# OpenGVLab/MM-Interleaved

Hardware: NVIDIA H100
Metric: interleaved_steps_per_sec (higher is better)
Workload: dtype bf16

## Files before the change

include/mmfs_b200.h:

```cpp
#ifndef MMFS_B200_H_
#define MMFS_B200_H_

#include <stdint.h>

#ifdef __cplusplus
extern "C" {
#endif

#define MMFS_B200_ABI_VERSION 3

#define MMFS_OK            0
#define MMFS_EINVAL       (-1)
#define MMFS_EUNSUPPORTED (-2)
#define MMFS_ECUDA        (-3)

#define MMFS_F32  0
#define MMFS_F16  1
#define MMFS_BF16 2
#define MMFS_F64  3

#define MMFS_MSDA_STRICT 1u

#define MMFS_SAMPLER_EXACT_WEIGHTS 4u
#define MMFS_SAMPLER_GENERIC       8u

int mmfs_abi_version(void);
const char *mmfs_last_error(void);

int mmfs_msda_forward(const void *value, const int64_t *spatial_shapes, const int64_t *level_start,
                      const void *sampling_loc, const void *attn_weight, void *out,
                      int N, int S, int M, int D, int L, int Lq, int P,
                      int dtype, unsigned flags, void *stream);

int mmfs_msda_backward(const void *value, const int64_t *spatial_shapes, const int64_t *level_start,
                       const void *sampling_loc, const void *attn_weight, const void *grad_out,
                       float *grad_value, float *grad_loc, float *grad_attn,
                       int N, int S, int M, int D, int L, int Lq, int P, int dtype, void *stream);

int mmfs_msda_backward_deterministic(const void *value, const int64_t *spatial_shapes, const int64_t *level_start,
                                     const void *sampling_loc, const void *attn_weight, const void *grad_out,
                                     long long *grad_value_fixed, float *grad_value, float *grad_loc, float *grad_attn,
                                     float *scratch2, int N, int S, int M, int D, int L, int Lq, int P, int dtype, void *stream);

int mmfs_msda_index_stream(const int64_t *spatial_shapes, const int64_t *level_start,
                           const void *sampling_loc, int32_t *idx,
                           int N, int M, int D, int L, int Lq, int P,
                           int dtype, void *stream);

int mmfs_msda_forward_host(const void *value, const int64_t *spatial_shapes, const int64_t *level_start,
                           const void *sampling_loc, const void *attn_weight, void *out,
                           int N, int S, int M, int D, int L, int Lq, int P,
                           int dtype, unsigned flags, void *stream);
void mmfs_release_scratch(void);

int mmfs_sampler_forward(const void *value, const int64_t *shapes, const int64_t *starts,
                         const void *qproj, const void *rtable, const uint8_t *relpos,
                         const float *refpts, const float *scale_ratios, void *out, float *null_mass,
                         int N, int S, int M, int D, int n_img, int n_lvl, int Lq, int P,
                         int Lq_r, int Nr, int Lr, int R, int dtype, unsigned flags, void *stream);

int mmfs_sampler_locw(const int64_t *shapes, const int64_t *starts, const void *qproj, const void *rtable,
                      const uint8_t *relpos, const float *refpts, const float *scale_ratios,
                      void *loc_out, void *attn_out, float *null_mass,
                      int N, int M, int n_img, int n_lvl, int Lq, int P,
                      int Lq_r, int Nr, int Lr, int R, int dtype, void *stream);

int mmfs_rmsnorm(const void *x, const void *weight, void *y, long rows, int cols, float eps, int dtype, void *stream);
int mmfs_layernorm(const void *x, const void *weight, const void *bias, void *y, long rows, int cols, float eps,
                   int dtype, void *stream);
int mmfs_rope_qk(void *q, void *k, const float *cos_table, const float *sin_table, const int64_t *position_ids,
                 long n_tokens, int T_len, int H, int hd, int q_stride, int k_stride, int pos_per_batch,
                 int dtype, void *stream);
int mmfs_rope_qk_append(void *q, const void *k, const void *v, const float *cos_table, const float *sin_table,
                        const int64_t *position_ids, void *k_cache, void *v_cache, const int64_t *slot_dev, long slot_host,
                        long n_tokens, int T_len, int H, int hd, int q_stride, int k_stride, int v_stride, long cache_bs,
                        long cache_ts, int pos_per_batch, int dtype, void *stream);
int mmfs_swiglu(const void *gate_up, void *out, long rows, int inter, int dtype, void *stream);
int mmfs_geglu(const void *value_gate, void *out, long rows, int inter, int dtype, void *stream);

int mmfs_attn_generic(const void *q, const void *k, const void *v, void *out, const uint8_t *key_mask,
                      int B, int H, int Tq, int Tkv, int hd,
                      long q_bs, long q_ts, long k_bs, long k_ts, long v_bs, long v_ts, long o_bs, long o_ts,
                      float scale, int causal, int past, int dtype, void *stream);
long mmfs_attn_decode_scratch_floats(int B, int H, int Tkv, int hd);
int mmfs_attn_decode(const void *q, const void *k, const void *v, void *out, const uint8_t *key_mask, float *scratch,
                     int B, int H, int Tkv, int hd, long q_bs, long k_bs, long k_ts, long v_bs, long v_ts, long o_bs,
                     float scale, int causal, int past, int dtype, void *stream);

int mmfs_attn_forward(const void *q, const void *k, const void *v, void *out, const uint8_t *key_mask,
                      int B, int H, int Tq, int Tkv, int hd,
                      long q_bs, long q_ts, long k_bs, long k_ts, long v_bs, long v_ts, long o_bs, long o_ts,
                      float scale, int causal, int past, int dtype, unsigned *work_counter, void *stream);

int mmfs_attn_forward_lse(const void *q, const void *k, const void *v, void *out, float *lse, const uint8_t *key_mask,
                          int B, int H, int Tq, int Tkv, int hd,
                          long q_bs, long q_ts, long k_bs, long k_ts, long v_bs, long v_ts, long o_bs, long o_ts,
                          float scale, int causal, int past, int dtype, unsigned *work_counter, void *stream);

int mmfs_attn_backward(const void *q, const void *k, const void *v, const void *out, const void *d_out, const float *lse,
                       void *dq, void *dk, void *dv, float *delta, const uint8_t *key_mask, int B, int H, int T, int hd,
                       long q_bs, long q_ts, long k_bs, long k_ts, long v_bs, long v_ts, long o_bs, long o_ts,
                       long do_bs, long do_ts, long dq_bs, long dq_ts, long dk_bs, long dk_ts, long dv_bs, long dv_ts,
                       float scale, int dtype, void *stream);

#define MMFS_RMSNORM_BWD_PARTS 256
int mmfs_rmsnorm_backward(const void *x, const void *weight, const void *dy, void *dx, void *dweight, float *partials,
                          long rows, int cols, float eps, int dtype, void *stream);

int mmfs_swiglu_backward(const void *gate_up, const void *d_out, void *d_gate_up, long rows, int inter, int dtype,
                         void *stream);

int mmfs_conv2d_nhwc(const void *x, const void *w, const void *bias, const void *add_bc, const void *residual, void *out,
                     int B, int H, int W, int Cin, int Cout, int KH, int KW, int stride, int pad, int dtype, void *stream);

int mmfs_conv2d_up2x_nhwc(const void *x, const void *w_phases, const void *bias, void *out, int B, int H, int W, int Cin,
                          int Cout, int dtype, void *stream);

int mmfs_conv2d_down2x_nhwc(const void *x, const void *w, const void *bias, void *out, int B, int H, int W, int Cin,
                            int Cout, int dtype, void *stream);

int mmfs_groupnorm_nhwc(const void *x, const void *gamma, const void *beta, void *y, float *stats, int B, int HW, int C,
                        int G, float eps, int silu, int dtype, void *stream);

#define MMFS_SELECT_GREEDY 0
#define MMFS_SELECT_SAMPLE 1

int mmfs_decode_select(const float *logits, long ld, int64_t *out_ids, const int64_t *step, uint8_t *finished,
                       int64_t *next_ids, const int64_t *eos_ids, int n_eos, long pad_id, int min_length,
                       const float *params, const int64_t *seed, const float *uniforms, int B, int V, int max_new,
                       int mode, void *stream);

int mmfs_beam_select(const float *logits, long ld, const int64_t *step, const double *params, float *beam_scores,
                     int64_t *history, int64_t *next_ids, int64_t *parent, uint8_t *done, double *hyp_scores,
                     int64_t *hyp_ids, int64_t *hyp_meta, const int64_t *eos_ids, int n_eos, long pad_id, int min_length,
                     uint64_t *scratch, int B, int num_beams, int V, int max_new, void *stream);

int mmfs_beam_sample(const float *logits, long ld, const int64_t *step, const double *params, const int64_t *seed,
                     const float *uniforms, float *beam_scores, int64_t *history, int64_t *next_ids, int64_t *parent,
                     uint8_t *done, double *hyp_scores, int64_t *hyp_ids, int64_t *hyp_meta, int32_t *error,
                     const int64_t *eos_ids, int n_eos, long pad_id, int min_length, int top_k, uint64_t *scratch, int B,
                     int num_beams, int V, int max_new, void *stream);

int mmfs_kv_beam_reorder(void *cache, int n_caches, long cache_stride, int rows, long row_stride, long pos_stride,
                         long row_bytes, int num_beams, const int64_t *parent, const int64_t *cur, const int64_t *step,
                         const uint8_t *done, int max_positions, void *stream);

#ifdef __cplusplus
}
#endif
#endif
```

mm-interleaved_b200/_lib.py:

```python
from __future__ import annotations

import ctypes
import os

_HERE = os.path.dirname(os.path.abspath(__file__))
LIB_PATH = os.environ.get("MMFS_B200_LIB", os.path.join(_HERE, "libmmfs_b200.so"))

OK, EINVAL, EUNSUPPORTED, ECUDA = 0, -1, -2, -3
F32, F16, BF16, F64 = 0, 1, 2, 3
MSDA_STRICT = 1
SAMPLER_EXACT_WEIGHTS = 4
SAMPLER_GENERIC = 8
SELECT_GREEDY, SELECT_SAMPLE = 0, 1

_lib = None

_I, _U, _P = ctypes.c_int, ctypes.c_uint, ctypes.c_void_p
_L, _F = ctypes.c_long, ctypes.c_float

SIGNATURES = {
    "mmfs_abi_version": (_I, []),
    "mmfs_last_error": (ctypes.c_char_p, []),
    "mmfs_msda_forward": (_I, [_P, _P, _P, _P, _P, _P, _I, _I, _I, _I, _I, _I, _I, _I, _U, _P]),
    "mmfs_msda_backward": (_I, [_P] * 9 + [_I] * 8 + [_P]),
    "mmfs_msda_backward_deterministic": (_I, [_P] * 11 + [_I] * 8 + [_P]),
    "mmfs_msda_index_stream": (_I, [_P, _P, _P, _P, _I, _I, _I, _I, _I, _I, _I, _P]),
    "mmfs_msda_forward_host": (_I, [_P, _P, _P, _P, _P, _P, _I, _I, _I, _I, _I, _I, _I, _I, _U, _P]),
    "mmfs_release_scratch": (None, []),
    "mmfs_sampler_forward": (_I, [_P] * 10 + [_I] * 13 + [_U, _P]),
    "mmfs_sampler_locw": (_I, [_P] * 10 + [_I] * 11 + [_P]),
    "mmfs_rmsnorm": (_I, [_P, _P, _P, _L, _I, _F, _I, _P]),
    "mmfs_layernorm": (_I, [_P, _P, _P, _P, _L, _I, _F, _I, _P]),
    "mmfs_rope_qk": (_I, [_P, _P, _P, _P, _P, _L, _I, _I, _I, _I, _I, _I, _I, _P]),
    "mmfs_rope_qk_append": (_I, [_P] * 9 + [_L, _L] + [_I] * 6 + [_L, _L, _I, _I, _P]),
    "mmfs_swiglu": (_I, [_P, _P, _L, _I, _I, _P]),
    "mmfs_geglu": (_I, [_P, _P, _L, _I, _I, _P]),
    "mmfs_attn_generic": (_I, [_P] * 5 + [_I] * 5 + [_L] * 8 + [_F, _I, _I, _I, _P]),
    "mmfs_groupnorm_nhwc": (_I, [_P] * 5 + [_I] * 4 + [_F, _I, _I, _P]),
    "mmfs_conv2d_nhwc": (_I, [_P] * 6 + [_I] * 10 + [_P]),
    "mmfs_conv2d_up2x_nhwc": (_I, [_P] * 4 + [_I] * 6 + [_P]),
    "mmfs_conv2d_down2x_nhwc": (_I, [_P] * 4 + [_I] * 6 + [_P]),
    "mmfs_attn_decode_scratch_floats": (_L, [_I] * 4),
    "mmfs_attn_decode": (_I, [_P] * 6 + [_I] * 4 + [_L] * 6 + [_F, _I, _I, _I, _P]),
    "mmfs_attn_forward": (_I, [_P] * 5 + [_I] * 5 + [_L] * 8 + [_F, _I, _I, _I, _P, _P]),
    "mmfs_attn_forward_lse": (_I, [_P] * 6 + [_I] * 5 + [_L] * 8 + [_F, _I, _I, _I, _P, _P]),
    "mmfs_attn_backward": (_I, [_P] * 11 + [_I] * 4 + [_L] * 16 + [_F, _I, _P]),
    "mmfs_rmsnorm_backward": (_I, [_P] * 6 + [_L, _I, _F, _I, _P]),
    "mmfs_swiglu_backward": (_I, [_P] * 3 + [_L, _I, _I, _P]),
    "mmfs_decode_select": (_I, [_P, _L] + [_P] * 5 + [_I, _L, _I] + [_P] * 3 + [_I] * 4 + [_P]),
    "mmfs_beam_select": (_I, [_P, _L] + [_P] * 11 + [_I, _L, _I, _P] + [_I] * 4 + [_P]),
    "mmfs_beam_sample": (_I, [_P, _L] + [_P] * 14 + [_I, _L, _I, _I, _P] + [_I] * 4 + [_P]),
    "mmfs_kv_beam_reorder": (_I, [_P, _I, _L, _I, _L, _L, _L, _I] + [_P] * 4 + [_I, _P]),
}
BEAM_MAX_BEAMS, BEAM_MAX_EOS = 8, 4
RMSNORM_BWD_PARTS = 256


def lib() -> ctypes.CDLL:
    global _lib
    if _lib is None:
        if not os.path.exists(LIB_PATH):
            raise RuntimeError(
                f"libmmfs_b200.so not found at {LIB_PATH}: build it with "
                "`python mm-interleaved_b200/build.py` (there is no CPU / PyTorch fallback)")
        handle = ctypes.CDLL(LIB_PATH)
        for name, (res, args) in SIGNATURES.items():
            fn = getattr(handle, name)
            fn.restype = res
            fn.argtypes = args
        if handle.mmfs_abi_version() != 3:
            raise RuntimeError(f"libmmfs_b200.so ABI {handle.mmfs_abi_version()} != 3")
        _lib = handle
    return _lib


def check(rc: int, what: str) -> None:
    if rc != OK:
        msg = lib().mmfs_last_error().decode("utf-8", "replace")
        kind = {EINVAL: "invalid argument", EUNSUPPORTED: "unsupported", ECUDA: "CUDA error"}.get(rc, "error")
        raise RuntimeError(f"{what}: {kind} ({rc}): {msg}")
```

mm-interleaved_b200/csrc/conv_igemm_sm100.cu:

```cuda
#include "tc_common.cuh"

namespace mmfs {

constexpr int kConvStages = 4;
constexpr int kConvThreads = 288;
constexpr int kConvConsumers = 256;

struct ConvParams {
    void *out;
    const void *bias, *add_bc, *residual;
    int B, Ho, Wo, Cin, Cout, KH, KW, stride, pad;
    int TW, TH, TB;
    int tiles_w, tiles_h;
};

template <typename T> __device__ __forceinline__ uint32_t cpack2(float a, float b);
template <> __device__ __forceinline__ uint32_t cpack2<__nv_bfloat16>(float a, float b) {
    __nv_bfloat162 t = __floats2bfloat162_rn(a, b);
    return *reinterpret_cast<uint32_t *>(&t);
}
template <> __device__ __forceinline__ uint32_t cpack2<__half>(float a, float b) {
    __half2 t = __floats2half2_rn(a, b);
    return *reinterpret_cast<uint32_t *>(&t);
}
template <typename T> __device__ __forceinline__ float2 cunpack2(const T *p);
template <> __device__ __forceinline__ float2 cunpack2<__nv_bfloat16>(const __nv_bfloat16 *p) {
    return __bfloat1622float2(*reinterpret_cast<const __nv_bfloat162 *>(p));
}
template <> __device__ __forceinline__ float2 cunpack2<__half>(const __half *p) {
    return __half22float2(*reinterpret_cast<const __half2 *>(p));
}

template <typename T, int BN, bool UP>
__global__ void __launch_bounds__(kConvThreads, 1)
conv_igemm_kernel(const __grid_constant__ CUtensorMap map_x, const __grid_constant__ CUtensorMap map_w, const ConvParams p) {
    static_assert(BN == 160 || BN == 128, "Cout tile");
    constexpr uint32_t A_BYTES = 128 * 128, B_BYTES = BN * 128, STAGE_BYTES = A_BYTES + B_BYTES;
    extern __shared__ __align__(1024) uint8_t smem_raw[];
    if ((s_addr(smem_raw) & 1023u) != 0u) { asm volatile("trap;"); }
    uint64_t *bars = reinterpret_cast<uint64_t *>(smem_raw + kConvStages * STAGE_BYTES);
    uint64_t *full = bars, *empty = bars + kConvStages;

    const int warp = threadIdx.x >> 5, lane = threadIdx.x & 31;
    int t = blockIdx.x;
    const int wt = t % p.tiles_w; t /= p.tiles_w;
    const int ht = t % p.tiles_h; t /= p.tiles_h;
    const int b0 = t * p.TB, h0 = ht * p.TH, w0 = wt * p.TW;
    const int n0 = blockIdx.y * BN;
    const int kc = p.Cin / 64;
    const int n_k = p.KH * p.KW * kc;

    if (threadIdx.x == 0) {
        for (int i = 0; i < kConvStages; ++i) { bar_init(full + i, 1); bar_init(empty + i, kConvConsumers); }
        asm volatile("fence.mbarrier_init.release.cluster;" ::: "memory");
    }
    __syncthreads();

    if (warp == 8) {
        if (lane == 0) {
            for (int it = 0; it < n_k; ++it) {
                const int s = it % kConvStages;
                const uint32_t ph = (it / kConvStages) & 1;
                bar_wait(empty + s, ph ^ 1);
                const int tap = it / kc, cb = it - tap * kc;
                const int kh = tap / p.KW, kw = tap - kh * p.KW;
                uint8_t *sa = smem_raw + s * STAGE_BYTES;
                bar_expect_tx(full + s, STAGE_BYTES);
                if constexpr (UP) {
                    const int phase = blockIdx.z;
                    tma_load_4d(sa, &map_x, full + s, cb * 64, w0 + kw - 1 + (phase & 1), h0 + kh - 1 + (phase >> 1), b0);
                    tma_load_2d(sa + A_BYTES, &map_w, full + s, tap * p.Cin + cb * 64, phase * p.Cout + n0);
                } else {
                    tma_load_4d(sa, &map_x, full + s, cb * 64, w0 * p.stride + kw - p.pad, h0 * p.stride + kh - p.pad, b0);
                    tma_load_2d(sa + A_BYTES, &map_w, full + s, tap * p.Cin + cb * 64, n0);
                }
            }
        }
        return;
    }

    const int wg = warp >> 2;
    float acc[BN / 2];
#pragma unroll
    for (int i = 0; i < BN / 2; ++i) acc[i] = 0.f;
    for (int it = 0; it < n_k; ++it) {
        const int s = it % kConvStages;
        bar_wait(full + s, (it / kConvStages) & 1);
        const uint32_t sa = s_addr(smem_raw) + s * STAGE_BYTES;
        reg_fence(acc);
        wgmma_fence();
#pragma unroll
        for (int kk = 0; kk < 4; ++kk) {
            const uint64_t da = smem_desc(sa + wg * 64 * 128 + kk * 32, 16, 1024), db = smem_desc(sa + A_BYTES + kk * 32, 16, 1024);
            if constexpr (BN == 160) Wgmma<T>::ss_n160(acc, da, db, 1);
            else Wgmma<T>::ss_n128(acc, da, db, 1);
        }
        wgmma_commit();
        wgmma_wait<1>();
        reg_fence(acc);
        if (it > 0) bar_arrive(empty + (it - 1) % kConvStages);
    }
    wgmma_wait<0>();
    reg_fence(acc);

    const int tq = lane & 3;
    const T *bp = p.bias ? static_cast<const T *>(p.bias) + n0 + 2 * tq : nullptr;
#pragma unroll
    for (int i = 0; i < 2; ++i) {
        const int row = wg * 64 + (warp & 3) * 16 + (lane >> 2) + 8 * i;
        const int pw = row % p.TW, phh = (row / p.TW) % p.TH, pb = row / (p.TW * p.TH);
        const int b = b0 + pb, ho = h0 + phh, wo = w0 + pw;
        if (b >= p.B || ho >= p.Ho || wo >= p.Wo) continue;
        size_t pix;
        if constexpr (UP) pix = ((size_t)b * 2 * p.Ho + 2 * ho + (blockIdx.z >> 1)) * 2 * p.Wo + 2 * wo + (blockIdx.z & 1);
        else pix = ((size_t)b * p.Ho + ho) * p.Wo + wo;
        T *op = static_cast<T *>(p.out) + pix * p.Cout + n0 + 2 * tq;
        const T *rp = p.residual ? static_cast<const T *>(p.residual) + pix * p.Cout + n0 + 2 * tq : nullptr;
        const T *ap = p.add_bc ? static_cast<const T *>(p.add_bc) + (size_t)b * p.Cout + n0 + 2 * tq : nullptr;
#pragma unroll
        for (int j = 0; j < BN / 8; ++j) {
            float e0 = acc[j * 4 + 2 * i], e1 = acc[j * 4 + 2 * i + 1];
            if (bp) { const float2 f = cunpack2<T>(bp + j * 8); e0 += f.x; e1 += f.y; }
            if (ap) { const float2 f = cunpack2<T>(ap + j * 8); e0 += f.x; e1 += f.y; }
            if (rp) { const float2 f = cunpack2<T>(rp + j * 8); e0 += f.x; e1 += f.y; }
            *reinterpret_cast<uint32_t *>(op + j * 8) = cpack2<T>(e0, e1);
        }
    }
}

}

using namespace mmfs;

namespace {

int conv_bn(int Cout) { return Cout % 160 == 0 ? 160 : Cout % 128 == 0 ? 128 : 0; }

template <auto kern>
int launch(dim3 grid, size_t smem, cudaStream_t st, const CUtensorMap &mx, const CUtensorMap &mw, const ConvParams &p) {
    const int rc = ensure_dynamic_smem<kern>(smem);
    if (rc != MMFS_OK) return rc;
    kern<<<grid, kConvThreads, smem, st>>>(mx, mw, p);
    MMFS_CUDA(cudaGetLastError());
    return MMFS_OK;
}

template <bool UP>
int launch_conv(const char *what, const void *x, const void *w, const void *bias, const void *add_bc, const void *residual,
                void *out, int B, int H, int W, int Ho, int Wo, int Cin, int Cout, int KH, int KW, int stride, int pad,
                int dtype, void *stream) {
    int TW, TH, TB;
    if (Wo % 16 == 0 && Ho % 8 == 0) { TW = 16; TH = 8; TB = 1; }
    else if (Wo == 8 && Ho == 8 && B % 2 == 0) { TW = 8; TH = 8; TB = 2; }
    else { set_error("%s: output %dx%d (B=%d) is not tileable by the 128-pixel patches", what, Ho, Wo, B); return MMFS_EUNSUPPORTED; }
    const int BN = conv_bn(Cout);
    if (!(dtype == MMFS_BF16 || dtype == MMFS_F16) || Cin % 64 != 0 || BN == 0 || stride > 2 ||
        ((uintptr_t)x | (uintptr_t)w | (uintptr_t)out | (uintptr_t)bias | (uintptr_t)add_bc | (uintptr_t)residual) % 16 != 0) {
        set_error("%s: needs bf16/f16, Cin %% 64 == 0, Cout %% 160 == 0 or Cout %% 128 == 0, stride <= 2, 16-byte aligned "
                  "pointers (Cin=%d Cout=%d)", what, Cin, Cout);
        return MMFS_EUNSUPPORTED;
    }
    EncodeTiledFn enc = tensor_map_encoder();
    if (!enc) { set_error("%s: cuTensorMapEncodeTiled unavailable", what); return MMFS_ECUDA; }
    const CUtensorMapDataType dt = dtype == MMFS_BF16 ? CU_TENSOR_MAP_DATA_TYPE_BFLOAT16 : CU_TENSOR_MAP_DATA_TYPE_FLOAT16;
    const int phases = UP ? 4 : 1;
    CUtensorMap mx, mw;
    {
        const cuuint64_t dims[4] = {(cuuint64_t)Cin, (cuuint64_t)W, (cuuint64_t)H, (cuuint64_t)B};
        const cuuint64_t strides[3] = {(cuuint64_t)Cin * 2, (cuuint64_t)W * Cin * 2, (cuuint64_t)H * W * Cin * 2};
        const cuuint32_t box[4] = {64, (cuuint32_t)(TW * stride), (cuuint32_t)(TH * stride), (cuuint32_t)TB};
        const cuuint32_t estr[4] = {1, (cuuint32_t)stride, (cuuint32_t)stride, 1};
        CUresult r = enc(&mx, dt, 4, const_cast<void *>(x), dims, strides, box, estr, CU_TENSOR_MAP_INTERLEAVE_NONE,
                         CU_TENSOR_MAP_SWIZZLE_128B, CU_TENSOR_MAP_L2_PROMOTION_L2_128B, CU_TENSOR_MAP_FLOAT_OOB_FILL_NONE);
        if (r != CUDA_SUCCESS) { set_error("%s: tensor map (input) failed (%d)", what, (int)r); return MMFS_ECUDA; }
    }
    {
        const cuuint64_t K = (cuuint64_t)KH * KW * Cin;
        const cuuint64_t dims[2] = {K, (cuuint64_t)Cout * phases};
        const cuuint64_t strides[1] = {K * 2};
        const cuuint32_t box[2] = {64, (cuuint32_t)BN};
        const cuuint32_t estr[2] = {1, 1};
        CUresult r = enc(&mw, dt, 2, const_cast<void *>(w), dims, strides, box, estr, CU_TENSOR_MAP_INTERLEAVE_NONE,
                         CU_TENSOR_MAP_SWIZZLE_128B, CU_TENSOR_MAP_L2_PROMOTION_L2_256B, CU_TENSOR_MAP_FLOAT_OOB_FILL_NONE);
        if (r != CUDA_SUCCESS) { set_error("%s: tensor map (weights) failed (%d)", what, (int)r); return MMFS_ECUDA; }
    }
    ConvParams p;
    p.out = out; p.bias = bias; p.add_bc = add_bc; p.residual = residual;
    p.B = B; p.Ho = Ho; p.Wo = Wo; p.Cin = Cin; p.Cout = Cout; p.KH = KH; p.KW = KW; p.stride = stride; p.pad = pad;
    p.TW = TW; p.TH = TH; p.TB = TB; p.tiles_w = Wo / TW; p.tiles_h = Ho / TH;
    const size_t smem = (size_t)kConvStages * (128 * 128 + BN * 128) + 2 * kConvStages * 8;
    dim3 grid((unsigned)(p.tiles_w * p.tiles_h * (B / TB)), (unsigned)(Cout / BN), (unsigned)phases);
    cudaStream_t st = (cudaStream_t)stream;
    return dispatch_dtype<kF16Types>(dtype, what, [&](auto tag) {
        using T = typename decltype(tag)::type;
        return BN == 160 ? launch<conv_igemm_kernel<T, 160, UP>>(grid, smem, st, mx, mw, p)
                         : launch<conv_igemm_kernel<T, 128, UP>>(grid, smem, st, mx, mw, p);
    });
}

}

extern "C" int mmfs_conv2d_nhwc(const void *x, const void *w, const void *bias, const void *add_bc, const void *residual, void *out,
                                int B, int H, int W, int Cin, int Cout, int KH, int KW, int stride, int pad,
                                int dtype, void *stream) {
    MMFS_CHECK_ARG(B > 0 && H > 0 && W > 0 && Cin > 0 && Cout > 0 && KH > 0 && KW > 0 && stride > 0 && pad >= 0, "conv2d_nhwc: bad dimension");
    MMFS_CHECK_ARG(x && w && out, "conv2d_nhwc: null pointer argument");
    const int Ho = (H + 2 * pad - KH) / stride + 1, Wo = (W + 2 * pad - KW) / stride + 1;
    return launch_conv<false>("conv2d_nhwc", x, w, bias, add_bc, residual, out, B, H, W, Ho, Wo, Cin, Cout, KH, KW, stride,
                              pad, dtype, stream);
}

extern "C" int mmfs_conv2d_up2x_nhwc(const void *x, const void *w_phases, const void *bias, void *out, int B, int H, int W, int Cin,
                                     int Cout, int dtype, void *stream) {
    MMFS_CHECK_ARG(B > 0 && H > 0 && W > 0 && Cin > 0 && Cout > 0, "conv2d_up2x_nhwc: bad dimension");
    MMFS_CHECK_ARG(x && w_phases && out, "conv2d_up2x_nhwc: null pointer argument");
    return launch_conv<true>("conv2d_up2x_nhwc", x, w_phases, bias, nullptr, nullptr, out, B, H, W, H, W, Cin, Cout, 2, 2, 1, 0,
                             dtype, stream);
}

extern "C" int mmfs_conv2d_down2x_nhwc(const void *x, const void *w, const void *bias, void *out, int B, int H, int W, int Cin,
                                       int Cout, int dtype, void *stream) {
    MMFS_CHECK_ARG(B > 0 && H > 0 && W > 0 && Cin > 0 && Cout > 0, "conv2d_down2x_nhwc: bad dimension");
    MMFS_CHECK_ARG(x && w && out, "conv2d_down2x_nhwc: null pointer argument");
    MMFS_CHECK_ARG(H % 2 == 0 && W % 2 == 0, "conv2d_down2x_nhwc: odd H or W");
    return launch_conv<false>("conv2d_down2x_nhwc", x, w, bias, nullptr, nullptr, out, B, H, W, H / 2, W / 2, Cin, Cout, 3, 3,
                              2, 0, dtype, stream);
}
```

mm-interleaved_b200/csrc/llama_ops_sm100.cu:

```cuda
#include "common.cuh"

namespace mmfs {

template <typename T> __device__ __forceinline__ float rnd(float x) { return to_op(from_op<T>(x)); }
template <> __device__ __forceinline__ float rnd<float>(float x) { return x; }

__device__ __forceinline__ float block_sum(float v, float *s_red) {
#pragma unroll
    for (int o = 16; o > 0; o >>= 1) v += __shfl_xor_sync(0xffffffffu, v, o);
    const int lane = threadIdx.x & 31, warp = threadIdx.x >> 5, nw = (blockDim.x + 31) >> 5;
    if (lane == 0) s_red[warp] = v;
    __syncthreads();
    float t = (lane < nw) ? s_red[lane] : 0.f;
#pragma unroll
    for (int o = 16; o > 0; o >>= 1) t += __shfl_xor_sync(0xffffffffu, t, o);
    __syncthreads();
    return t;
}

template <typename T>
__global__ void __launch_bounds__(256) rmsnorm_kernel(const T *__restrict__ x, const T *__restrict__ w,
                                                       T *__restrict__ y, int cols, float eps) {
    constexpr int VEC = 16 / (int)sizeof(T);
    __shared__ float s_red[32];
    const size_t row = blockIdx.x;
    const T *xr = x + row * cols;
    T *yr = y + row * cols;
    const int nvec = cols / VEC;
    float ss = 0.f;
    for (int i = threadIdx.x; i < nvec; i += blockDim.x) {
        float f[VEC];
        Vec16<T>::unpack(*reinterpret_cast<const uint4 *>(xr + i * VEC), f);
#pragma unroll
        for (int k = 0; k < VEC; ++k) ss += f[k] * f[k];
    }
    for (int i = nvec * VEC + threadIdx.x; i < cols; i += blockDim.x) { const float v = to_op(xr[i]); ss += v * v; }
    const float var = block_sum(ss, s_red) / (float)cols;
    const float r = rsqrtf(var + eps);
    for (int i = threadIdx.x; i < nvec; i += blockDim.x) {
        float f[VEC], g[VEC], o[VEC];
        Vec16<T>::unpack(*reinterpret_cast<const uint4 *>(xr + i * VEC), f);
        Vec16<T>::unpack(*reinterpret_cast<const uint4 *>(w + i * VEC), g);
#pragma unroll
        for (int k = 0; k < VEC; ++k) o[k] = g[k] * rnd<T>(f[k] * r);
        *reinterpret_cast<uint4 *>(yr + i * VEC) = Vec16<T>::pack(o);
    }
    for (int i = nvec * VEC + threadIdx.x; i < cols; i += blockDim.x)
        yr[i] = from_op<T>(to_op(w[i]) * rnd<T>(to_op(xr[i]) * r));
}

constexpr int kRmsChunks = 8;
constexpr int kRmsThreads = 128;

template <typename T>
__global__ void __launch_bounds__(kRmsThreads) rmsnorm_reg_kernel(const T *__restrict__ x, const T *__restrict__ w,
                                                                  T *__restrict__ y, int cols, float eps) {
    constexpr int VEC = 16 / (int)sizeof(T);
    __shared__ float s_red[kRmsThreads / 32];
    const size_t row = blockIdx.x;
    const T *xr = x + row * cols;
    T *yr = y + row * cols;
    const int nvec = cols / VEC;
    uint4 v[kRmsChunks], wv[kRmsChunks];
#pragma unroll
    for (int c = 0; c < kRmsChunks; ++c) {
        const int i = threadIdx.x + c * kRmsThreads;
        if (i < nvec) {
            v[c] = ldg_nc_v4(xr + i * VEC);
            wv[c] = ldg_nc_v4(w + i * VEC);
        }
    }
    float ss = 0.f;
#pragma unroll
    for (int c = 0; c < kRmsChunks; ++c)
        if (threadIdx.x + c * kRmsThreads < nvec) {
            float f[VEC];
            Vec16<T>::unpack(v[c], f);
#pragma unroll
            for (int k = 0; k < VEC; ++k) ss = fmaf(f[k], f[k], ss);
        }
#pragma unroll
    for (int o = 16; o > 0; o >>= 1) ss += __shfl_xor_sync(0xffffffffu, ss, o);
    if ((threadIdx.x & 31) == 0) s_red[threadIdx.x >> 5] = ss;
    __syncthreads();
    float tot = 0.f;
#pragma unroll
    for (int i = 0; i < kRmsThreads / 32; ++i) tot += s_red[i];
    const float r = rsqrtf(tot / (float)cols + eps);
#pragma unroll
    for (int c = 0; c < kRmsChunks; ++c) {
        const int i = threadIdx.x + c * kRmsThreads;
        if (i < nvec) {
            float f[VEC], g[VEC], o[VEC];
            Vec16<T>::unpack(v[c], f);
            Vec16<T>::unpack(wv[c], g);
#pragma unroll
            for (int k = 0; k < VEC; ++k) o[k] = g[k] * rnd<T>(f[k] * r);
            stg_v4(yr + i * VEC, Vec16<T>::pack(o));
        }
    }
}

constexpr int kLnChunks = 8;

template <typename T, int CH>
__global__ void __launch_bounds__(256, CH == 8 ? 2 : 4) layernorm_warp_kernel(const T *__restrict__ x, const T *__restrict__ w,
                                                              const T *__restrict__ b, T *__restrict__ y, long rows, int cols, float eps) {
    constexpr int VEC = 16 / (int)sizeof(T);
    const int lane = threadIdx.x & 31;
    const long row = (long)blockIdx.x * (blockDim.x >> 5) + (threadIdx.x >> 5);
    if (row >= rows) return;
    const T *xr = x + row * cols;
    T *yr = y + row * cols;
    const int nvec = cols / VEC;
    uint4 v[CH];
#pragma unroll
    for (int c = 0; c < CH; ++c) {
        const int i = lane + 32 * c;
        v[c] = (i < nvec) ? ldg_nc_v4(xr + i * VEC) : make_uint4(0u, 0u, 0u, 0u);
    }
    float s = 0.f;
#pragma unroll
    for (int c = 0; c < CH; ++c) {
        float f[VEC];
        Vec16<T>::unpack(v[c], f);
#pragma unroll
        for (int k = 0; k < VEC; ++k) s += f[k];
    }
#pragma unroll
    for (int o = 16; o > 0; o >>= 1) s += __shfl_xor_sync(0xffffffffu, s, o);
    const float mean = s / (float)cols;
    float ss = 0.f;
#pragma unroll
    for (int c = 0; c < CH; ++c)
        if (lane + 32 * c < nvec) {
            float f[VEC];
            Vec16<T>::unpack(v[c], f);
#pragma unroll
            for (int k = 0; k < VEC; ++k) { const float d = f[k] - mean; ss = fmaf(d, d, ss); }
        }
#pragma unroll
    for (int o = 16; o > 0; o >>= 1) ss += __shfl_xor_sync(0xffffffffu, ss, o);
    const float r = rsqrtf(ss / (float)cols + eps);
#pragma unroll
    for (int c = 0; c < CH; ++c) {
        const int i = lane + 32 * c;
        if (i < nvec) {
            float f[VEC], g[VEC], bb[VEC], o[VEC];
            Vec16<T>::unpack(v[c], f);
            if (w) Vec16<T>::unpack(*reinterpret_cast<const uint4 *>(w + i * VEC), g);
            if (b) Vec16<T>::unpack(*reinterpret_cast<const uint4 *>(b + i * VEC), bb);
#pragma unroll
            for (int k = 0; k < VEC; ++k) o[k] = (f[k] - mean) * r * (w ? g[k] : 1.f) + (b ? bb[k] : 0.f);
            stg_v4(yr + i * VEC, Vec16<T>::pack(o));
        }
    }
}

template <typename T>
__global__ void __launch_bounds__(256) layernorm_kernel(const T *__restrict__ x, const T *__restrict__ w,
                                                         const T *__restrict__ b, T *__restrict__ y, int cols, float eps) {
    __shared__ float s_red[32];
    const size_t row = blockIdx.x;
    const T *xr = x + row * cols;
    T *yr = y + row * cols;
    float s = 0.f;
    for (int i = threadIdx.x; i < cols; i += blockDim.x) s += to_op(xr[i]);
    const float mean = block_sum(s, s_red) / (float)cols;
    float ss = 0.f;
    for (int i = threadIdx.x; i < cols; i += blockDim.x) { const float d = to_op(xr[i]) - mean; ss += d * d; }
    const float r = rsqrtf(block_sum(ss, s_red) / (float)cols + eps);
    for (int i = threadIdx.x; i < cols; i += blockDim.x) {
        const float n = (to_op(xr[i]) - mean) * r;
        yr[i] = from_op<T>(n * (w ? to_op(w[i]) : 1.f) + (b ? to_op(b[i]) : 0.f));
    }
}

template <typename T>
__global__ void __launch_bounds__(256) rope_qk_kernel(T *__restrict__ q, T *__restrict__ k, const float *__restrict__ cos_t,
                                                       const float *__restrict__ sin_t, const int64_t *__restrict__ pos,
                                                       long n_tok, int H, int hd, int q_stride, int k_stride, int pos_per_batch,
                                                       int T_len) {
    constexpr int VEC = 16 / (int)sizeof(T);
    const int half = hd >> 1;
    const int chunks = half / VEC;
    const int per_tok = 2 * H * chunks;
    const bool hoist = (blockDim.x % chunks) == 0;
    for (long tok = blockIdx.x; tok < n_tok; tok += gridDim.x) {
        const long p = pos[pos_per_batch ? tok : (tok % T_len)];
        const float *cp = cos_t + p * hd, *sp = sin_t + p * hd;
        T *qt = q + tok * q_stride, *kt = k + tok * k_stride;
        float cs[VEC], sn[VEC];
        auto load_table = [&](int c) {
#pragma unroll
            for (int i = 0; i < VEC; i += 4) {
                const float4 a = *reinterpret_cast<const float4 *>(cp + c * VEC + i);
                const float4 b = *reinterpret_cast<const float4 *>(sp + c * VEC + i);
                cs[i] = rnd<T>(a.x); cs[i + 1] = rnd<T>(a.y); cs[i + 2] = rnd<T>(a.z); cs[i + 3] = rnd<T>(a.w);
                sn[i] = rnd<T>(b.x); sn[i + 1] = rnd<T>(b.y); sn[i + 2] = rnd<T>(b.z); sn[i + 3] = rnd<T>(b.w);
            }
        };
        if (hoist) load_table(threadIdx.x % chunks);
        for (int it = threadIdx.x; it < per_tok; it += blockDim.x) {
            const int c = it % chunks;
            const int hh = it / chunks;
            T *x = (hh >= H ? kt + (size_t)(hh - H) * hd : qt + (size_t)hh * hd) + c * VEC;
            float x1[VEC], x2[VEC], o1[VEC], o2[VEC];
            const uint4 v1 = *reinterpret_cast<const uint4 *>(x), v2 = *reinterpret_cast<const uint4 *>(x + half);
            if (!hoist) load_table(c);
            Vec16<T>::unpack(v1, x1);
            Vec16<T>::unpack(v2, x2);
#pragma unroll
            for (int i = 0; i < VEC; ++i) {
                o1[i] = rnd<T>(x1[i] * cs[i]) + rnd<T>(-x2[i] * sn[i]);
                o2[i] = rnd<T>(x2[i] * cs[i]) + rnd<T>(x1[i] * sn[i]);
            }
            *reinterpret_cast<uint4 *>(x) = Vec16<T>::pack(o1);
            *reinterpret_cast<uint4 *>(x + half) = Vec16<T>::pack(o2);
        }
    }
}

template <typename T>
__global__ void __launch_bounds__(256) rope_append_kernel(T *__restrict__ q, const T *__restrict__ k, const T *__restrict__ v,
                                                           const float *__restrict__ cos_t, const float *__restrict__ sin_t,
                                                           const int64_t *__restrict__ pos, T *__restrict__ k_cache,
                                                           T *__restrict__ v_cache, const int64_t *__restrict__ slot_dev,
                                                           long slot_host, long n_tok, int H, int hd, int q_stride, int k_stride,
                                                           int v_stride, long cache_bs, long cache_ts, int pos_per_batch, int T_len) {
    constexpr int VEC = 16 / (int)sizeof(T);
    const int half = hd >> 1;
    const int chunks = half / VEC;
    const int n_rot = 2 * H * chunks;
    const int n_copy = H * hd / VEC;
    const long slot = slot_dev != nullptr ? (long)*slot_dev : slot_host;
    for (long tok = blockIdx.x; tok < n_tok; tok += gridDim.x) {
        const long p = pos[pos_per_batch ? tok : (tok % T_len)];
        const float *cp = cos_t + p * hd, *sp = sin_t + p * hd;
        const long b = tok / T_len, tt = tok - b * T_len;
        T *qt = q + tok * q_stride;
        const T *kt = k + tok * k_stride, *vt = v + tok * v_stride;
        T *kc = k_cache + b * cache_bs + (slot + tt) * cache_ts, *vc = v_cache + b * cache_bs + (slot + tt) * cache_ts;
        for (int it = threadIdx.x; it < n_rot + n_copy; it += blockDim.x) {
            if (it >= n_rot) {
                const int i = (it - n_rot) * VEC;
                *reinterpret_cast<uint4 *>(vc + i) = *reinterpret_cast<const uint4 *>(vt + i);
                continue;
            }
            const int c = it % chunks, hh = it / chunks;
            const bool is_k = hh >= H;
            const T *src = (is_k ? kt + (size_t)(hh - H) * hd : qt + (size_t)hh * hd) + c * VEC;
            T *dst = (is_k ? kc + (size_t)(hh - H) * hd : qt + (size_t)hh * hd) + c * VEC;
            float cs[VEC], sn[VEC], x1[VEC], x2[VEC], o1[VEC], o2[VEC];
#pragma unroll
            for (int i = 0; i < VEC; i += 4) {
                const float4 a = *reinterpret_cast<const float4 *>(cp + c * VEC + i);
                const float4 bb = *reinterpret_cast<const float4 *>(sp + c * VEC + i);
                cs[i] = rnd<T>(a.x); cs[i + 1] = rnd<T>(a.y); cs[i + 2] = rnd<T>(a.z); cs[i + 3] = rnd<T>(a.w);
                sn[i] = rnd<T>(bb.x); sn[i + 1] = rnd<T>(bb.y); sn[i + 2] = rnd<T>(bb.z); sn[i + 3] = rnd<T>(bb.w);
            }
            Vec16<T>::unpack(*reinterpret_cast<const uint4 *>(src), x1);
            Vec16<T>::unpack(*reinterpret_cast<const uint4 *>(src + half), x2);
#pragma unroll
            for (int i = 0; i < VEC; ++i) {
                o1[i] = rnd<T>(x1[i] * cs[i]) + rnd<T>(-x2[i] * sn[i]);
                o2[i] = rnd<T>(x2[i] * cs[i]) + rnd<T>(x1[i] * sn[i]);
            }
            *reinterpret_cast<uint4 *>(dst) = Vec16<T>::pack(o1);
            *reinterpret_cast<uint4 *>(dst + half) = Vec16<T>::pack(o2);
        }
    }
}

template <typename T> __device__ __forceinline__ float silu_op(float g) { return __fdividef(g, 1.f + __expf(-g)); }
template <> __device__ __forceinline__ float silu_op<float>(float g) { return g / (1.f + expf(-g)); }

template <typename T, int ACT> __device__ __forceinline__ float glu_act(float g) {
    if (ACT == 0) return silu_op<T>(g);
    return 0.5f * g * (1.f + erff(g * 0.70710678118654752f));
}

template <typename T, int ACT = 0, bool GATE_SECOND = false>
__global__ void __launch_bounds__(256) swiglu_kernel(const T *__restrict__ gu, T *__restrict__ out, long rows, int I) {
    constexpr int VEC = 16 / (int)sizeof(T);
    const int per = (I / VEC + gridDim.y - 1) / gridDim.y;
    const int v0 = blockIdx.y * per, nvec = min(I / VEC, v0 + per);
    for (long r = blockIdx.x; r < rows; r += gridDim.x) {
        const T *g_row = gu + r * 2 * I + (GATE_SECOND ? I : 0), *u_row = gu + r * 2 * I + (GATE_SECOND ? 0 : I);
        T *o_row = out + r * I;
        int i = v0 + threadIdx.x;
        for (; i + (int)blockDim.x < nvec; i += 2 * blockDim.x) {
            const int j = i + blockDim.x;
            const uint4 g0 = ldg_nc_v4(g_row + i * VEC), u0 = ldg_nc_v4(u_row + i * VEC);
            const uint4 g1 = ldg_nc_v4(g_row + j * VEC), u1 = ldg_nc_v4(u_row + j * VEC);
            float g[VEC], u[VEC], o[VEC];
            Vec16<T>::unpack(g0, g); Vec16<T>::unpack(u0, u);
#pragma unroll
            for (int k = 0; k < VEC; ++k) o[k] = rnd<T>(glu_act<T, ACT>(g[k])) * u[k];
            stg_v4(o_row + i * VEC, Vec16<T>::pack(o));
            Vec16<T>::unpack(g1, g); Vec16<T>::unpack(u1, u);
#pragma unroll
            for (int k = 0; k < VEC; ++k) o[k] = rnd<T>(glu_act<T, ACT>(g[k])) * u[k];
            stg_v4(o_row + j * VEC, Vec16<T>::pack(o));
        }
        if (i < nvec) {
            float g[VEC], u[VEC], o[VEC];
            Vec16<T>::unpack(ldg_nc_v4(g_row + i * VEC), g); Vec16<T>::unpack(ldg_nc_v4(u_row + i * VEC), u);
#pragma unroll
            for (int k = 0; k < VEC; ++k) o[k] = rnd<T>(glu_act<T, ACT>(g[k])) * u[k];
            stg_v4(o_row + i * VEC, Vec16<T>::pack(o));
        }
    }
}

template <typename T>
static int launch_rmsnorm(const void *x, const void *w, void *y, long rows, int cols, float eps, cudaStream_t st) {
    if (cols % (16 / (int)sizeof(T)) == 0 && cols / (16 / (int)sizeof(T)) <= kRmsThreads * kRmsChunks)
        rmsnorm_reg_kernel<T><<<(unsigned)rows, kRmsThreads, 0, st>>>((const T *)x, (const T *)w, (T *)y, cols, eps);
    else
        rmsnorm_kernel<T><<<(unsigned)rows, 256, 0, st>>>((const T *)x, (const T *)w, (T *)y, cols, eps);
    MMFS_CUDA(cudaGetLastError());
    return MMFS_OK;
}

template <typename T>
static int launch_layernorm(const void *x, const void *w, const void *b, void *y, long rows, int cols, float eps, cudaStream_t st) {
    constexpr int VEC = 16 / (int)sizeof(T);
    const bool vec_ok = (cols % VEC == 0) && (cols / VEC <= 32 * kLnChunks) &&
                        (((uintptr_t)x | (uintptr_t)y | (uintptr_t)w | (uintptr_t)b) % 16 == 0);
    if (vec_ok) {
        const int nvec = cols / VEC;
        const unsigned grid = (unsigned)((rows + 7) / 8);
#define MMFS_LN(CH) layernorm_warp_kernel<T, CH><<<grid, 256, 0, st>>>((const T *)x, (const T *)w, (const T *)b, (T *)y, rows, cols, eps)
        if (nvec <= 32) MMFS_LN(1); else if (nvec <= 64) MMFS_LN(2); else if (nvec <= 128) MMFS_LN(4); else MMFS_LN(8);
#undef MMFS_LN
    } else
        layernorm_kernel<T><<<(unsigned)rows, 256, 0, st>>>((const T *)x, (const T *)w, (const T *)b, (T *)y, cols, eps);
    MMFS_CUDA(cudaGetLastError());
    return MMFS_OK;
}

template <typename T>
static int launch_rope(void *q, void *k, const float *cos_t, const float *sin_t, const int64_t *pos, long n_tok, int T_len,
                       int H, int hd, int qs, int ks, int ppb, cudaStream_t st) {
    const int per_tok = H * 2 * ((hd / 2) / (16 / (int)sizeof(T)));
    const int threads = per_tok >= 256 ? 256 : ((per_tok + 31) / 32) * 32;
    rope_qk_kernel<T><<<capped_grid(n_tok, 32), threads, 0, st>>>((T *)q, (T *)k, cos_t, sin_t, pos, n_tok, H, hd, qs, ks, ppb,
                                                                  T_len);
    MMFS_CUDA(cudaGetLastError());
    return MMFS_OK;
}

template <typename T>
static int launch_glu(const void *in, void *out, long rows, int inter, bool geglu, cudaStream_t st) {
    const int nvec = inter / (16 / (int)sizeof(T));
    const int threads = nvec >= 512 ? 256 : (nvec >= 64 ? 64 : 32);
    const int gx = capped_grid(rows, 64);
    int gy = 1;
    if (gx < num_sms()) { gy = (nvec + 2 * threads - 1) / (2 * threads); if (gy > 64) gy = 64; if (gy < 1) gy = 1; }
    const dim3 grid(gx, gy);
    if (geglu)
        swiglu_kernel<T, 1, true><<<grid, threads, 0, st>>>((const T *)in, (T *)out, rows, inter);
    else
        swiglu_kernel<T, 0, false><<<grid, threads, 0, st>>>((const T *)in, (T *)out, rows, inter);
    MMFS_CUDA(cudaGetLastError());
    return MMFS_OK;
}

template <typename T>
static int launch_rope_append(void *q, const void *k, const void *v, const float *cos_t, const float *sin_t, const int64_t *pos,
                              void *kc, void *vc, const int64_t *slot_dev, long slot_host, long n_tok, int T_len, int H, int hd,
                              int qs, int ks, int vs, long cbs, long cts, int ppb, cudaStream_t st) {
    const int items = H * ((hd / 2) / (16 / (int)sizeof(T))) * 2 + H * hd / (16 / (int)sizeof(T));
    const int threads = items >= 256 ? 256 : ((items + 31) / 32) * 32;
    rope_append_kernel<T><<<capped_grid(n_tok, 32), threads, 0, st>>>((T *)q, (const T *)k, (const T *)v, cos_t, sin_t, pos, (T *)kc,
                                                                      (T *)vc, slot_dev, slot_host, n_tok, H, hd, qs, ks, vs, cbs,
                                                                      cts, ppb, T_len);
    MMFS_CUDA(cudaGetLastError());
    return MMFS_OK;
}


constexpr int kRmsBwdParts = MMFS_RMSNORM_BWD_PARTS;
constexpr int kRmsBwdMaxCols = 8192;

template <typename T>
__global__ void __launch_bounds__(256) rmsnorm_bwd_kernel(const T *__restrict__ x, const T *__restrict__ w,
                                                          const T *__restrict__ dy, T *__restrict__ dx,
                                                          float *__restrict__ partials, long rows, int cols, float eps) {
    constexpr int VEC = 16 / (int)sizeof(T);
    extern __shared__ float s_dw[];
    __shared__ float s_red[32];
    const int nvec = cols / VEC;
    if (partials)
        for (int i = threadIdx.x; i < nvec; i += blockDim.x)
#pragma unroll
            for (int k = 0; k < VEC; ++k) s_dw[i * VEC + k] = 0.f;
    for (long row = blockIdx.x; row < rows; row += gridDim.x) {
        const T *xr = x + row * cols, *dyr = dy + row * cols;
        float ss = 0.f, sg = 0.f;
        for (int i = threadIdx.x; i < nvec; i += blockDim.x) {
            float f[VEC], g[VEC], d[VEC];
            Vec16<T>::unpack(ldg_nc_v4(xr + i * VEC), f);
            Vec16<T>::unpack(ldg_nc_v4(w + i * VEC), g);
            Vec16<T>::unpack(ldg_nc_v4(dyr + i * VEC), d);
#pragma unroll
            for (int k = 0; k < VEC; ++k) { ss = fmaf(f[k], f[k], ss); sg = fmaf(d[k] * g[k], f[k], sg); }
        }
        ss = block_sum(ss, s_red);
        sg = block_sum(sg, s_red);
        const float r = rsqrtf(ss / (float)cols + eps);
        const float coef = r * r * r * sg / (float)cols;
        for (int i = threadIdx.x; i < nvec; i += blockDim.x) {
            float f[VEC], g[VEC], d[VEC], o[VEC];
            Vec16<T>::unpack(ldg_nc_v4(xr + i * VEC), f);
            Vec16<T>::unpack(ldg_nc_v4(w + i * VEC), g);
            Vec16<T>::unpack(ldg_nc_v4(dyr + i * VEC), d);
#pragma unroll
            for (int k = 0; k < VEC; ++k) o[k] = fmaf(r * d[k], g[k], -f[k] * coef);
            stg_v4(dx + row * cols + i * VEC, Vec16<T>::pack(o));
            if (partials)
#pragma unroll
                for (int k = 0; k < VEC; ++k) s_dw[i * VEC + k] = fmaf(d[k], rnd<T>(f[k] * r), s_dw[i * VEC + k]);
        }
    }
    if (partials)
        for (int i = threadIdx.x; i < nvec; i += blockDim.x)
#pragma unroll
            for (int k = 0; k < VEC; ++k) partials[(long)blockIdx.x * cols + i * VEC + k] = s_dw[i * VEC + k];
}

template <typename T>
__global__ void __launch_bounds__(256) rmsnorm_dw_reduce_kernel(const float *__restrict__ partials, T *__restrict__ dw,
                                                                int parts, int cols) {
    const int c = blockIdx.x * blockDim.x + threadIdx.x;
    if (c >= cols) return;
    float s = 0.f;
    for (int p = 0; p < parts; ++p) s += partials[(long)p * cols + c];
    dw[c] = from_op<T>(s);
}

template <typename T>
__global__ void __launch_bounds__(256) swiglu_bwd_kernel(const T *__restrict__ gu, const T *__restrict__ d_out,
                                                         T *__restrict__ d_gu, long rows, int I) {
    constexpr int VEC = 16 / (int)sizeof(T);
    const int nvec = I / VEC;
    for (long r = blockIdx.x; r < rows; r += gridDim.x)
        for (int i = threadIdx.x; i < nvec; i += blockDim.x) {
            float g[VEC], u[VEC], d[VEC], dg[VEC], du[VEC];
            Vec16<T>::unpack(ldg_nc_v4(gu + r * 2 * I + i * VEC), g);
            Vec16<T>::unpack(ldg_nc_v4(gu + r * 2 * I + I + i * VEC), u);
            Vec16<T>::unpack(ldg_nc_v4(d_out + r * I + i * VEC), d);
#pragma unroll
            for (int k = 0; k < VEC; ++k) {
                const float s = 1.f / (1.f + expf(-g[k]));
                dg[k] = d[k] * u[k] * s * fmaf(g[k], 1.f - s, 1.f);
                du[k] = d[k] * g[k] * s;
            }
            stg_v4(d_gu + r * 2 * I + i * VEC, Vec16<T>::pack(dg));
            stg_v4(d_gu + r * 2 * I + I + i * VEC, Vec16<T>::pack(du));
        }
}

template <typename T>
static int launch_rmsnorm_bwd(const void *x, const void *w, const void *dy, void *dx, void *dw, float *partials, long rows,
                              int cols, float eps, cudaStream_t st) {
    const int parts = (int)(rows < kRmsBwdParts ? rows : kRmsBwdParts);
    rmsnorm_bwd_kernel<T><<<parts, 256, dw ? cols * sizeof(float) : 0, st>>>(
        (const T *)x, (const T *)w, (const T *)dy, (T *)dx, dw ? partials : nullptr, rows, cols, eps);
    MMFS_CUDA(cudaGetLastError());
    if (dw) {
        rmsnorm_dw_reduce_kernel<T><<<(cols + 255) / 256, 256, 0, st>>>(partials, (T *)dw, parts, cols);
        MMFS_CUDA(cudaGetLastError());
    }
    return MMFS_OK;
}

template <typename T>
static int launch_swiglu_bwd(const void *gu, const void *d_out, void *d_gu, long rows, int inter, cudaStream_t st) {
    swiglu_bwd_kernel<T><<<capped_grid(rows, 8), 256, 0, st>>>((const T *)gu, (const T *)d_out, (T *)d_gu, rows, inter);
    MMFS_CUDA(cudaGetLastError());
    return MMFS_OK;
}

}

using namespace mmfs;

extern "C" int mmfs_rmsnorm(const void *x, const void *weight, void *y, long rows, int cols, float eps, int dtype, void *stream) {
    MMFS_CHECK_ARG(rows >= 0 && cols > 0, "rmsnorm: bad shape");
    if (rows == 0) return MMFS_OK;
    MMFS_CHECK_ARG(x && weight && y, "rmsnorm: null pointer argument");
    MMFS_CHECK_ARG(((uintptr_t)x | (uintptr_t)weight | (uintptr_t)y) % 16 == 0 && (cols * dtype_size(dtype)) % 16 == 0,
                   "rmsnorm: rows must be 16-byte aligned");
    return dispatch_dtype<kF32Types>(dtype, "rmsnorm", [&](auto tag) {
        return launch_rmsnorm<typename decltype(tag)::type>(x, weight, y, rows, cols, eps, (cudaStream_t)stream);
    });
}

extern "C" int mmfs_layernorm(const void *x, const void *weight, const void *bias, void *y, long rows, int cols, float eps,
                              int dtype, void *stream) {
    MMFS_CHECK_ARG(rows >= 0 && cols > 0, "layernorm: bad shape");
    if (rows == 0) return MMFS_OK;
    MMFS_CHECK_ARG(x && y, "layernorm: null pointer argument");
    return dispatch_dtype<kF32Types>(dtype, "layernorm", [&](auto tag) {
        return launch_layernorm<typename decltype(tag)::type>(x, weight, bias, y, rows, cols, eps, (cudaStream_t)stream);
    });
}

extern "C" int mmfs_rope_qk(void *q, void *k, const float *cos_table, const float *sin_table, const int64_t *position_ids,
                            long n_tokens, int T_len, int H, int hd, int q_stride, int k_stride, int pos_per_batch,
                            int dtype, void *stream) {
    MMFS_CHECK_ARG(n_tokens >= 0 && H > 0 && hd > 0 && hd % 2 == 0 && T_len > 0, "rope_qk: bad shape");
    if (n_tokens == 0) return MMFS_OK;
    MMFS_CHECK_ARG(q && k && cos_table && sin_table && position_ids, "rope_qk: null pointer argument");
    MMFS_CHECK_ARG((hd / 2) % (16 / (int)dtype_size(dtype)) == 0 && ((uintptr_t)q | (uintptr_t)k) % 16 == 0 &&
                   (q_stride * dtype_size(dtype)) % 16 == 0 && (k_stride * dtype_size(dtype)) % 16 == 0,
                   "rope_qk: head_dim/2 must be a multiple of the 16-byte vector and rows 16-byte aligned");
    return dispatch_dtype<kF32Types>(dtype, "rope_qk", [&](auto tag) {
        return launch_rope<typename decltype(tag)::type>(q, k, cos_table, sin_table, position_ids, n_tokens, T_len, H, hd, q_stride,
                                                         k_stride, pos_per_batch, (cudaStream_t)stream);
    });
}

extern "C" int mmfs_rope_qk_append(void *q, const void *k, const void *v, const float *cos_table, const float *sin_table,
                                   const int64_t *position_ids, void *k_cache, void *v_cache, const int64_t *slot_dev,
                                   long slot_host, long n_tokens, int T_len, int H, int hd, int q_stride, int k_stride,
                                   int v_stride, long cache_bs, long cache_ts, int pos_per_batch, int dtype, void *stream) {
    MMFS_CHECK_ARG(n_tokens >= 0 && H > 0 && hd > 0 && hd % 2 == 0 && T_len > 0 && slot_host >= 0, "rope_qk_append: bad shape");
    if (n_tokens == 0) return MMFS_OK;
    MMFS_CHECK_ARG(q && k && v && cos_table && sin_table && position_ids && k_cache && v_cache, "rope_qk_append: null pointer argument");
    const size_t es = dtype_size(dtype);
    MMFS_CHECK_ARG(es == 2 || es == 4, "rope_qk_append: f32 / f16 / bf16");
    MMFS_CHECK_ARG((hd / 2) % (16 / (int)es) == 0 &&
                       ((uintptr_t)q | (uintptr_t)k | (uintptr_t)v | (uintptr_t)k_cache | (uintptr_t)v_cache) % 16 == 0 &&
                       (q_stride * es) % 16 == 0 && (k_stride * es) % 16 == 0 && (v_stride * es) % 16 == 0 &&
                       (cache_bs * es) % 16 == 0 && (cache_ts * es) % 16 == 0,
                   "rope_qk_append: head_dim/2 must be a multiple of the 16-byte vector and all rows 16-byte aligned");
    return dispatch_dtype<kF32Types>(dtype, "rope_qk_append", [&](auto tag) {
        return launch_rope_append<typename decltype(tag)::type>(q, k, v, cos_table, sin_table, position_ids, k_cache, v_cache,
                                                                slot_dev, slot_host, n_tokens, T_len, H, hd, q_stride, k_stride,
                                                                v_stride, cache_bs, cache_ts, pos_per_batch, (cudaStream_t)stream);
    });
}

extern "C" int mmfs_swiglu(const void *gate_up, void *out, long rows, int inter, int dtype, void *stream) {
    MMFS_CHECK_ARG(rows >= 0 && inter > 0, "swiglu: bad shape");
    if (rows == 0) return MMFS_OK;
    MMFS_CHECK_ARG(gate_up && out, "swiglu: null pointer argument");
    MMFS_CHECK_ARG(((uintptr_t)gate_up | (uintptr_t)out) % 16 == 0 && (inter * dtype_size(dtype)) % 16 == 0,
                   "swiglu: rows must be 16-byte aligned");
    return dispatch_dtype<kF32Types>(dtype, "swiglu", [&](auto tag) {
        return launch_glu<typename decltype(tag)::type>(gate_up, out, rows, inter, false, (cudaStream_t)stream);
    });
}

extern "C" int mmfs_geglu(const void *value_gate, void *out, long rows, int inter, int dtype, void *stream) {
    MMFS_CHECK_ARG(rows >= 0 && inter > 0, "geglu: bad shape");
    if (rows == 0) return MMFS_OK;
    MMFS_CHECK_ARG(value_gate && out, "geglu: null pointer argument");
    MMFS_CHECK_ARG(((uintptr_t)value_gate | (uintptr_t)out) % 16 == 0 && (inter * dtype_size(dtype)) % 16 == 0,
                   "geglu: rows must be 16-byte aligned");
    return dispatch_dtype<kF32Types>(dtype, "geglu", [&](auto tag) {
        return launch_glu<typename decltype(tag)::type>(value_gate, out, rows, inter, true, (cudaStream_t)stream);
    });
}

extern "C" int mmfs_rmsnorm_backward(const void *x, const void *weight, const void *dy, void *dx, void *dweight,
                                     float *partials, long rows, int cols, float eps, int dtype, void *stream) {
    MMFS_CHECK_ARG(rows >= 0 && cols > 0, "rmsnorm_backward: bad shape");
    if (rows == 0) return MMFS_OK;
    MMFS_CHECK_ARG(x && weight && dy && dx && (!dweight || partials), "rmsnorm_backward: null pointer argument");
    if (!(dtype == MMFS_BF16 || dtype == MMFS_F16) || cols % 8 != 0 || cols > kRmsBwdMaxCols ||
        ((uintptr_t)x | (uintptr_t)weight | (uintptr_t)dy | (uintptr_t)dx) % 16 != 0) {
        set_error("rmsnorm_backward: needs bf16 / f16, cols %% 8 == 0, cols <= %d, 16-byte aligned rows (got cols=%d dtype=%d)",
                  kRmsBwdMaxCols, cols, dtype);
        return MMFS_EUNSUPPORTED;
    }
    return dispatch_dtype<kF16Types, MMFS_EUNSUPPORTED>(dtype, "rmsnorm_backward", [&](auto tag) {
        return launch_rmsnorm_bwd<typename decltype(tag)::type>(x, weight, dy, dx, dweight, partials, rows, cols, eps,
                                                                (cudaStream_t)stream);
    });
}

extern "C" int mmfs_swiglu_backward(const void *gate_up, const void *d_out, void *d_gate_up, long rows, int inter, int dtype,
                                    void *stream) {
    MMFS_CHECK_ARG(rows >= 0 && inter > 0, "swiglu_backward: bad shape");
    if (rows == 0) return MMFS_OK;
    MMFS_CHECK_ARG(gate_up && d_out && d_gate_up, "swiglu_backward: null pointer argument");
    if (!(dtype == MMFS_BF16 || dtype == MMFS_F16) || inter % 8 != 0 ||
        ((uintptr_t)gate_up | (uintptr_t)d_out | (uintptr_t)d_gate_up) % 16 != 0) {
        set_error("swiglu_backward: needs bf16 / f16, inter %% 8 == 0 and 16-byte aligned rows (got inter=%d dtype=%d)", inter, dtype);
        return MMFS_EUNSUPPORTED;
    }
    return dispatch_dtype<kF16Types, MMFS_EUNSUPPORTED>(dtype, "swiglu_backward", [&](auto tag) {
        return launch_swiglu_bwd<typename decltype(tag)::type>(gate_up, d_out, d_gate_up, rows, inter, (cudaStream_t)stream);
    });
}
```

mm-interleaved_b200/csrc/tc_common.cuh:

```cuda
#pragma once
#include <cuda.h>

#include "common.cuh"

namespace mmfs {

__device__ __forceinline__ void tma_load_4d(void *dst, const CUtensorMap *map, uint64_t *bar, int c0, int c1, int c2, int c3) {
    asm volatile(
        "cp.async.bulk.tensor.4d.shared::cluster.global.mbarrier::complete_tx::bytes [%0], [%1, {%3, %4, %5, %6}], [%2];" ::
        "r"(s_addr(dst)), "l"(map), "r"(s_addr(bar)), "r"(c0), "r"(c1), "r"(c2), "r"(c3) : "memory");
}
__device__ __forceinline__ void fence_async_smem() { asm volatile("fence.proxy.async.shared::cta;" ::: "memory"); }

__device__ __forceinline__ void wgmma_fence() { asm volatile("wgmma.fence.sync.aligned;" ::: "memory"); }
__device__ __forceinline__ void wgmma_commit() { asm volatile("wgmma.commit_group.sync.aligned;" ::: "memory"); }
template <int N> __device__ __forceinline__ void wgmma_wait() { asm volatile("wgmma.wait_group.sync.aligned %0;" ::"n"(N) : "memory"); }
template <int N> __device__ __forceinline__ void reg_fence(float (&d)[N]) {
#pragma unroll
    for (int i = 0; i < N; ++i) asm volatile("" : "+f"(d[i])::"memory");
}

__device__ __forceinline__ uint64_t smem_desc(uint32_t saddr, uint32_t lbo_bytes, uint32_t sbo_bytes) {
    return (uint64_t)((saddr >> 4) & 0x3fffu) | ((uint64_t)((lbo_bytes >> 4) & 0x3fffu) << 16) |
           ((uint64_t)((sbo_bytes >> 4) & 0x3fffu) << 32) | (1ull << 62);
}

template <typename T> struct Wgmma;
#define MMFS_WGMMA_OPS(TY) \
     \
    __device__ __forceinline__ static void ss_n64(float (&d)[32], uint64_t da, uint64_t db, int acc) { \
        asm volatile( \
            "{\n\t.reg .pred p;\n\tsetp.ne.b32 p, %34, 0;\n\t" \
            "wgmma.mma_async.sync.aligned.m64n64k16.f32." TY "." TY " {%0,%1,%2,%3,%4,%5,%6,%7,%8,%9,%10,%11,%12,%13,%14,%15,%16,%17,%18,%19,%20,%21,%22,%23,%24,%25,%26,%27,%28,%29,%30,%31}, %32, %33, p, 1, 1, 0, 0;\n\t}" \
            : "+f"(d[0]), "+f"(d[1]), "+f"(d[2]), "+f"(d[3]), "+f"(d[4]), "+f"(d[5]), "+f"(d[6]), "+f"(d[7]), "+f"(d[8]), "+f"(d[9]), "+f"(d[10]), "+f"(d[11]), "+f"(d[12]), "+f"(d[13]), "+f"(d[14]), "+f"(d[15]), "+f"(d[16]), "+f"(d[17]), "+f"(d[18]), "+f"(d[19]), "+f"(d[20]), "+f"(d[21]), "+f"(d[22]), "+f"(d[23]), "+f"(d[24]), "+f"(d[25]), "+f"(d[26]), "+f"(d[27]), "+f"(d[28]), "+f"(d[29]), "+f"(d[30]), "+f"(d[31]) \
            : "l"(da), "l"(db), "r"(acc)); \
    } \
     \
    __device__ __forceinline__ static void ss_n128(float (&d)[64], uint64_t da, uint64_t db, int acc) { \
        asm volatile( \
            "{\n\t.reg .pred p;\n\tsetp.ne.b32 p, %66, 0;\n\t" \
            "wgmma.mma_async.sync.aligned.m64n128k16.f32." TY "." TY " {%0,%1,%2,%3,%4,%5,%6,%7,%8,%9,%10,%11,%12,%13,%14,%15,%16,%17,%18,%19,%20,%21,%22,%23,%24,%25,%26,%27,%28,%29,%30,%31,%32,%33,%34,%35,%36,%37,%38,%39,%40,%41,%42,%43,%44,%45,%46,%47,%48,%49,%50,%51,%52,%53,%54,%55,%56,%57,%58,%59,%60,%61,%62,%63}, %64, %65, p, 1, 1, 0, 0;\n\t}" \
            : "+f"(d[0]), "+f"(d[1]), "+f"(d[2]), "+f"(d[3]), "+f"(d[4]), "+f"(d[5]), "+f"(d[6]), "+f"(d[7]), "+f"(d[8]), "+f"(d[9]), "+f"(d[10]), "+f"(d[11]), "+f"(d[12]), "+f"(d[13]), "+f"(d[14]), "+f"(d[15]), "+f"(d[16]), "+f"(d[17]), "+f"(d[18]), "+f"(d[19]), "+f"(d[20]), "+f"(d[21]), "+f"(d[22]), "+f"(d[23]), "+f"(d[24]), "+f"(d[25]), "+f"(d[26]), "+f"(d[27]), "+f"(d[28]), "+f"(d[29]), "+f"(d[30]), "+f"(d[31]), "+f"(d[32]), "+f"(d[33]), "+f"(d[34]), "+f"(d[35]), "+f"(d[36]), "+f"(d[37]), "+f"(d[38]), "+f"(d[39]), "+f"(d[40]), "+f"(d[41]), "+f"(d[42]), "+f"(d[43]), "+f"(d[44]), "+f"(d[45]), "+f"(d[46]), "+f"(d[47]), "+f"(d[48]), "+f"(d[49]), "+f"(d[50]), "+f"(d[51]), "+f"(d[52]), "+f"(d[53]), "+f"(d[54]), "+f"(d[55]), "+f"(d[56]), "+f"(d[57]), "+f"(d[58]), "+f"(d[59]), "+f"(d[60]), "+f"(d[61]), "+f"(d[62]), "+f"(d[63]) \
            : "l"(da), "l"(db), "r"(acc)); \
    } \
     \
    __device__ __forceinline__ static void ss_n160(float (&d)[80], uint64_t da, uint64_t db, int acc) { \
        asm volatile( \
            "{\n\t.reg .pred p;\n\tsetp.ne.b32 p, %82, 0;\n\t" \
            "wgmma.mma_async.sync.aligned.m64n160k16.f32." TY "." TY " {%0,%1,%2,%3,%4,%5,%6,%7,%8,%9,%10,%11,%12,%13,%14,%15,%16,%17,%18,%19,%20,%21,%22,%23,%24,%25,%26,%27,%28,%29,%30,%31,%32,%33,%34,%35,%36,%37,%38,%39,%40,%41,%42,%43,%44,%45,%46,%47,%48,%49,%50,%51,%52,%53,%54,%55,%56,%57,%58,%59,%60,%61,%62,%63,%64,%65,%66,%67,%68,%69,%70,%71,%72,%73,%74,%75,%76,%77,%78,%79}, %80, %81, p, 1, 1, 0, 0;\n\t}" \
            : "+f"(d[0]), "+f"(d[1]), "+f"(d[2]), "+f"(d[3]), "+f"(d[4]), "+f"(d[5]), "+f"(d[6]), "+f"(d[7]), "+f"(d[8]), "+f"(d[9]), "+f"(d[10]), "+f"(d[11]), "+f"(d[12]), "+f"(d[13]), "+f"(d[14]), "+f"(d[15]), "+f"(d[16]), "+f"(d[17]), "+f"(d[18]), "+f"(d[19]), "+f"(d[20]), "+f"(d[21]), "+f"(d[22]), "+f"(d[23]), "+f"(d[24]), "+f"(d[25]), "+f"(d[26]), "+f"(d[27]), "+f"(d[28]), "+f"(d[29]), "+f"(d[30]), "+f"(d[31]), "+f"(d[32]), "+f"(d[33]), "+f"(d[34]), "+f"(d[35]), "+f"(d[36]), "+f"(d[37]), "+f"(d[38]), "+f"(d[39]), "+f"(d[40]), "+f"(d[41]), "+f"(d[42]), "+f"(d[43]), "+f"(d[44]), "+f"(d[45]), "+f"(d[46]), "+f"(d[47]), "+f"(d[48]), "+f"(d[49]), "+f"(d[50]), "+f"(d[51]), "+f"(d[52]), "+f"(d[53]), "+f"(d[54]), "+f"(d[55]), "+f"(d[56]), "+f"(d[57]), "+f"(d[58]), "+f"(d[59]), "+f"(d[60]), "+f"(d[61]), "+f"(d[62]), "+f"(d[63]), "+f"(d[64]), "+f"(d[65]), "+f"(d[66]), "+f"(d[67]), "+f"(d[68]), "+f"(d[69]), "+f"(d[70]), "+f"(d[71]), "+f"(d[72]), "+f"(d[73]), "+f"(d[74]), "+f"(d[75]), "+f"(d[76]), "+f"(d[77]), "+f"(d[78]), "+f"(d[79]) \
            : "l"(da), "l"(db), "r"(acc)); \
    } \
     \
    __device__ __forceinline__ static void rs_n64(float (&d)[32], const uint32_t (&a)[4], uint64_t db, int acc) { \
        asm volatile( \
            "{\n\t.reg .pred p;\n\tsetp.ne.b32 p, %37, 0;\n\t" \
            "wgmma.mma_async.sync.aligned.m64n64k16.f32." TY "." TY " {%0,%1,%2,%3,%4,%5,%6,%7,%8,%9,%10,%11,%12,%13,%14,%15,%16,%17,%18,%19,%20,%21,%22,%23,%24,%25,%26,%27,%28,%29,%30,%31}, {%32,%33,%34,%35}, %36, p, 1, 1, 1;\n\t}" \
            : "+f"(d[0]), "+f"(d[1]), "+f"(d[2]), "+f"(d[3]), "+f"(d[4]), "+f"(d[5]), "+f"(d[6]), "+f"(d[7]), "+f"(d[8]), "+f"(d[9]), "+f"(d[10]), "+f"(d[11]), "+f"(d[12]), "+f"(d[13]), "+f"(d[14]), "+f"(d[15]), "+f"(d[16]), "+f"(d[17]), "+f"(d[18]), "+f"(d[19]), "+f"(d[20]), "+f"(d[21]), "+f"(d[22]), "+f"(d[23]), "+f"(d[24]), "+f"(d[25]), "+f"(d[26]), "+f"(d[27]), "+f"(d[28]), "+f"(d[29]), "+f"(d[30]), "+f"(d[31]) \
            : "r"(a[0]), "r"(a[1]), "r"(a[2]), "r"(a[3]), "l"(db), "r"(acc)); \
    } \
     \
    __device__ __forceinline__ static void rs_n128(float (&d)[64], const uint32_t (&a)[4], uint64_t db, int acc) { \
        asm volatile( \
            "{\n\t.reg .pred p;\n\tsetp.ne.b32 p, %69, 0;\n\t" \
            "wgmma.mma_async.sync.aligned.m64n128k16.f32." TY "." TY " {%0,%1,%2,%3,%4,%5,%6,%7,%8,%9,%10,%11,%12,%13,%14,%15,%16,%17,%18,%19,%20,%21,%22,%23,%24,%25,%26,%27,%28,%29,%30,%31,%32,%33,%34,%35,%36,%37,%38,%39,%40,%41,%42,%43,%44,%45,%46,%47,%48,%49,%50,%51,%52,%53,%54,%55,%56,%57,%58,%59,%60,%61,%62,%63}, {%64,%65,%66,%67}, %68, p, 1, 1, 1;\n\t}" \
            : "+f"(d[0]), "+f"(d[1]), "+f"(d[2]), "+f"(d[3]), "+f"(d[4]), "+f"(d[5]), "+f"(d[6]), "+f"(d[7]), "+f"(d[8]), "+f"(d[9]), "+f"(d[10]), "+f"(d[11]), "+f"(d[12]), "+f"(d[13]), "+f"(d[14]), "+f"(d[15]), "+f"(d[16]), "+f"(d[17]), "+f"(d[18]), "+f"(d[19]), "+f"(d[20]), "+f"(d[21]), "+f"(d[22]), "+f"(d[23]), "+f"(d[24]), "+f"(d[25]), "+f"(d[26]), "+f"(d[27]), "+f"(d[28]), "+f"(d[29]), "+f"(d[30]), "+f"(d[31]), "+f"(d[32]), "+f"(d[33]), "+f"(d[34]), "+f"(d[35]), "+f"(d[36]), "+f"(d[37]), "+f"(d[38]), "+f"(d[39]), "+f"(d[40]), "+f"(d[41]), "+f"(d[42]), "+f"(d[43]), "+f"(d[44]), "+f"(d[45]), "+f"(d[46]), "+f"(d[47]), "+f"(d[48]), "+f"(d[49]), "+f"(d[50]), "+f"(d[51]), "+f"(d[52]), "+f"(d[53]), "+f"(d[54]), "+f"(d[55]), "+f"(d[56]), "+f"(d[57]), "+f"(d[58]), "+f"(d[59]), "+f"(d[60]), "+f"(d[61]), "+f"(d[62]), "+f"(d[63]) \
            : "r"(a[0]), "r"(a[1]), "r"(a[2]), "r"(a[3]), "l"(db), "r"(acc)); \
    }
template <> struct Wgmma<__nv_bfloat16> { MMFS_WGMMA_OPS("bf16") };
template <> struct Wgmma<__half> { MMFS_WGMMA_OPS("f16") };
#undef MMFS_WGMMA_OPS


__device__ __forceinline__ void tma_load_2d(void *dst, const CUtensorMap *map, uint64_t *bar, int c0, int c1) {
    asm volatile(
        "cp.async.bulk.tensor.2d.shared::cluster.global.mbarrier::complete_tx::bytes [%0], [%1, {%3, %4}], [%2];" ::
        "r"(s_addr(dst)), "l"(map), "r"(s_addr(bar)), "r"(c0), "r"(c1) : "memory");
}

typedef CUresult (*EncodeTiledFn)(CUtensorMap *, CUtensorMapDataType, cuuint32_t, void *, const cuuint64_t *, const cuuint64_t *,
                                  const cuuint32_t *, const cuuint32_t *, CUtensorMapInterleave, CUtensorMapSwizzle,
                                  CUtensorMapL2promotion, CUtensorMapFloatOOBfill);

inline EncodeTiledFn tensor_map_encoder() {
    static EncodeTiledFn fn = nullptr;
    if (!fn) {
        void *ptr = nullptr;
        cudaDriverEntryPointQueryResult qres;
        if (cudaGetDriverEntryPoint("cuTensorMapEncodeTiled", &ptr, cudaEnableDefault, &qres) == cudaSuccess &&
            qres == cudaDriverEntryPointSuccess)
            fn = (EncodeTiledFn)ptr;
    }
    return fn;
}

}
```

mm-interleaved_b200/llama_mmfs.py:

```python
from __future__ import annotations

import math
from dataclasses import dataclass, field
from types import SimpleNamespace
from typing import List, Optional, Tuple

import torch
import torch.nn.functional as F
from torch import nn

import torch.utils.checkpoint

from . import autograd_ops, ops
from ._cache import SourceCache, WeightCache
from .mmfs import MMFS


@dataclass
class LlamaMMFSConfig:
    vocab_size: int = 32002
    hidden_size: int = 5120
    intermediate_size: int = 13824
    num_hidden_layers: int = 40
    num_attention_heads: int = 40
    hidden_act: str = "silu"
    max_position_embeddings: int = 2048
    rms_norm_eps: float = 1e-6
    pad_token_id: int = 0
    cross_attention_frequency: int = 4
    spatial_shapes: List[int] = field(default_factory=lambda: [32, 16, 8])
    image_embed_dim: int = 1024
    use_cache: bool = True


def records_grad(module, *tensors) -> bool:
    if not torch.is_grad_enabled():
        return False
    return (any(t is not None and torch.is_tensor(t) and t.requires_grad for t in tensors)
            or any(p.requires_grad for p in module.parameters()))


def check_training_dtype(what, t):
    if t.dtype not in (torch.bfloat16, torch.float16):
        raise RuntimeError(f"{what}: the backward kernels take bf16 / fp16 only (got {t.dtype}); cast the model, or run "
                           "under torch.no_grad()")


def _cat_weight(cat, linears):
    if any(l.weight.requires_grad for l in linears):
        return torch.cat([l.weight for l in linears], 0)
    return cat.get()


class LlamaRMSNorm(nn.Module):
    def __init__(self, hidden_size, eps=1e-6):
        super().__init__()
        self.weight = nn.Parameter(torch.ones(hidden_size))
        self.variance_epsilon = eps

    def forward(self, hidden_states):
        if records_grad(self, hidden_states):
            check_training_dtype("LlamaRMSNorm", hidden_states)
            return autograd_ops.rmsnorm(hidden_states, self.weight.to(hidden_states.dtype), self.variance_epsilon)
        return ops.rmsnorm(hidden_states.contiguous(), self.weight, self.variance_epsilon)


def rotary_tables(dim: int, max_pos: int, base: float = 10000.0, device=None):
    inv_freq = 1.0 / (base ** (torch.arange(0, dim, 2, device=device).float() / dim))
    t = torch.arange(max_pos, device=device, dtype=torch.float32)
    freqs = torch.outer(t, inv_freq)
    emb = torch.cat((freqs, freqs), dim=-1)
    return emb.cos().contiguous(), emb.sin().contiguous()


_ROPE_TABLES = {}


def shared_rotary_tables(dim: int, need_pos: int, min_pos: int, device):
    key = (str(device), dim)
    hit = _ROPE_TABLES.get(key)
    if hit is None or hit[0] < need_pos:
        n = max(min_pos, need_pos if hit is None else max(need_pos, 2 * hit[0]))
        hit = (n,) + rotary_tables(dim, n, device=device)
        _ROPE_TABLES[key] = hit
    return hit[1], hit[2]


class _CatWeight:

    def __init__(self, *linears):
        self.linears = linears
        self._cache = WeightCache()

    def get(self):
        ws = [l.weight for l in self.linears]
        return self._cache.get(ws, lambda: torch.cat(ws, 0).contiguous())


def _addmm_residual(residual, x, weight, inplace):
    r2 = residual.view(-1, residual.shape[-1])
    x2 = x.reshape(-1, x.shape[-1])
    if inplace:
        r2.addmm_(x2, weight.t())
        return residual
    return torch.addmm(r2, x2, weight.t()).view_as(residual)


class LlamaMLP(nn.Module):
    def __init__(self, hidden_size: int, intermediate_size: int, hidden_act: str):
        super().__init__()
        if hidden_act != "silu":
            raise NotImplementedError("only the SiLU gate of Llama is implemented")
        self.gate_proj = nn.Linear(hidden_size, intermediate_size, bias=False)
        self.down_proj = nn.Linear(intermediate_size, hidden_size, bias=False)
        self.up_proj = nn.Linear(hidden_size, intermediate_size, bias=False)
        self._gate_up = _CatWeight(self.gate_proj, self.up_proj)

    def forward(self, x, residual=None, inplace=False):
        if records_grad(self, x, residual):
            check_training_dtype("LlamaMLP", x)
            act = autograd_ops.swiglu(F.linear(x, _cat_weight(self._gate_up, (self.gate_proj, self.up_proj))))
            if residual is None:
                return self.down_proj(act)
            return _addmm_residual(residual, act, self.down_proj.weight, False)
        gu = F.linear(x, self._gate_up.get())
        act = ops.swiglu(gu)
        if residual is None:
            return self.down_proj(act)
        return _addmm_residual(residual, act, self.down_proj.weight, inplace)


class StaticKV:

    __slots__ = ("k", "v", "length", "slot")

    def __init__(self, batch, max_len, heads, head_dim, dtype, device):
        self.k = torch.empty((batch, max_len, heads, head_dim), dtype=dtype, device=device)
        self.v = torch.empty_like(self.k)
        self.length = 0
        self.slot = None

    @classmethod
    def over(cls, k, v) -> "StaticKV":
        c = cls.__new__(cls)
        c.k, c.v, c.length, c.slot = k, v, 0, None
        return c


class PreparedVision:

    __slots__ = ("raw_shape", "values")

    def __init__(self, raw_shape):
        self.raw_shape = tuple(raw_shape)
        self.values = {}


class LlamaAttention(nn.Module):
    def __init__(self, config: LlamaMMFSConfig):
        super().__init__()
        self.config = config
        self.hidden_size = config.hidden_size
        self.num_heads = config.num_attention_heads
        self.head_dim = self.hidden_size // self.num_heads
        self.max_position_embeddings = config.max_position_embeddings
        if self.head_dim * self.num_heads != self.hidden_size:
            raise ValueError("hidden_size must be divisible by num_heads")
        self.q_proj = nn.Linear(self.hidden_size, self.hidden_size, bias=False)
        self.k_proj = nn.Linear(self.hidden_size, self.hidden_size, bias=False)
        self.v_proj = nn.Linear(self.hidden_size, self.hidden_size, bias=False)
        self.o_proj = nn.Linear(self.hidden_size, self.hidden_size, bias=False)
        self._qkv = _CatWeight(self.q_proj, self.k_proj, self.v_proj)
        self._rope = None

    def rope_tables(self, device, need_pos):
        if self._rope is None or self._rope[0] != device or self._rope[1] < need_pos:
            cos, sin = shared_rotary_tables(self.head_dim, need_pos, self.max_position_embeddings, device)
            self._rope = (device, cos.shape[0], cos, sin)
        return self._rope[2], self._rope[3]

    def forward(self, hidden_states, attention_mask=None, position_ids=None, past_key_value=None,
                output_attentions=False, use_cache=False, residual=None, inplace=False):
        if output_attentions:
            raise NotImplementedError("attention probabilities are never materialised by the fused kernel")
        B, T, _ = hidden_states.shape
        H, hd = self.num_heads, self.head_dim
        if records_grad(self, hidden_states, residual):
            return self._forward_training(hidden_states, attention_mask, position_ids, past_key_value, use_cache, residual)
        qkv = F.linear(hidden_states, self._qkv.get()).view(B, T, 3, H, hd)
        q, k, v = qkv[:, :, 0], qkv[:, :, 1], qkv[:, :, 2]
        static = isinstance(past_key_value, StaticKV)
        past = 0 if past_key_value is None else (past_key_value.length if static else past_key_value[0].shape[1])
        if position_ids is None:
            position_ids = torch.arange(past, past + T, device=hidden_states.device)
        cos, sin = self.rope_tables(hidden_states.device, past + T)
        if static and past_key_value.slot is not None:
            if T != 1:
                raise RuntimeError("StaticKV.slot (graph decode) takes one token per step")
            ops.rope_qk_append_(q, k, v, cos, sin, position_ids, past_key_value.k, past_key_value.v, past_key_value.slot)
            k, v = past_key_value.k, past_key_value.v
            past = k.shape[1] - 1
            present = past_key_value
        elif static:
            if past + T > past_key_value.k.shape[1]:
                raise RuntimeError(f"StaticKV of {past_key_value.k.shape[1]} positions cannot take {past} + {T}")
            ops.rope_qk_append_(q, k, v, cos, sin, position_ids, past_key_value.k, past_key_value.v, past)
            past_key_value.length = past + T
            k, v = past_key_value.k[:, :past + T], past_key_value.v[:, :past + T]
            present = past_key_value
        else:
            ops.rope_qk_(q, k, cos, sin, position_ids)
            if past_key_value is not None:
                k = torch.cat([past_key_value[0], k], dim=1)
                v = torch.cat([past_key_value[1], v], dim=1)
            present = (k, v) if use_cache else None
        key_mask = None
        if attention_mask is not None:
            if attention_mask.dim() == 4:
                key_mask = attention_mask[:, 0, -1, :] > (torch.finfo(attention_mask.dtype).min / 2)
            else:
                key_mask = attention_mask
        ctx = ops.attention(q, k, v, key_mask=key_mask, causal=True, past=past)
        out = self.o_proj(ctx) if residual is None else _addmm_residual(residual, ctx, self.o_proj.weight, inplace)
        return out, None, present

    def _forward_training(self, hidden_states, attention_mask, position_ids, past_key_value, use_cache, residual):
        if past_key_value is not None or use_cache:
            raise RuntimeError("LlamaAttention under autograd runs the prefill without a KV cache: pass use_cache=False "
                               "and no past_key_values, or run under torch.no_grad()")
        check_training_dtype("LlamaAttention", hidden_states)
        if self.head_dim != 128:
            raise RuntimeError(f"LlamaAttention under autograd needs head dim 128 (the attention backward kernel's), "
                               f"got {self.head_dim}")
        B, T, _ = hidden_states.shape
        w = _cat_weight(self._qkv, (self.q_proj, self.k_proj, self.v_proj))
        qkv = F.linear(hidden_states, w).view(B, T, 3, self.num_heads, self.head_dim)
        if position_ids is None:
            position_ids = torch.arange(T, device=hidden_states.device)
        cos, sin = self.rope_tables(hidden_states.device, T)
        qkv = autograd_ops.rope_qkv(qkv, cos, sin, position_ids)
        key_mask = attention_mask
        if attention_mask is not None and attention_mask.dim() == 4:
            key_mask = attention_mask[:, 0, -1, :] > (torch.finfo(attention_mask.dtype).min / 2)
        ctx = autograd_ops.attention(qkv, key_mask)
        out = self.o_proj(ctx) if residual is None else _addmm_residual(residual, ctx, self.o_proj.weight, False)
        return out, None, None


class LlamaMMFSAttention(nn.Module):
    def __init__(self, config: LlamaMMFSConfig, layer_idx):
        super().__init__()
        self.layer_idx = layer_idx
        self.config = config
        self.spatial_shapes = [(s, s) for s in config.spatial_shapes]
        self.hidden_size = config.hidden_size
        self.vision_hidden_size = config.image_embed_dim
        self.gate = nn.Parameter(torch.tensor([0.0]))
        self.attn = MMFS(layer_idx=layer_idx, d_model=self.hidden_size, d_query=self.hidden_size,
                         d_value=self.vision_hidden_size, d_out=self.hidden_size,
                         n_levels=len(config.spatial_shapes), n_heads=16, n_points=8,
                         ratio=self.vision_hidden_size / self.hidden_size, offset_init_magnitude=3.0,
                         spatial_shapes=config.spatial_shapes, max_num_image_per_seq=50)
        self.norm1 = LlamaRMSNorm(config.hidden_size, eps=config.rms_norm_eps)
        self.norm2 = LlamaRMSNorm(self.vision_hidden_size, eps=config.rms_norm_eps)
        self._vision_cache = SourceCache()
        self._gated = WeightCache()
        self._geom_cache = {}

    def _geometry(self, device, n_img, hw, len_q):
        per_img = sum(h * w for h, w in self.spatial_shapes)
        if hw != per_img:
            raise RuntimeError(f"vision features have {hw} positions per image, expected {per_img}")
        key = ("s", device, n_img)
        if key not in self._geom_cache:
            ss = torch.tensor(self.spatial_shapes * n_img, dtype=torch.long)
            starts = torch.cat((ss.new_zeros((1,)), ss.prod(1).cumsum(0)[:-1]))
            self._geom_cache[key] = (ss.to(device), starts.to(device))
        rkey = ("r", device, len_q)
        if rkey not in self._geom_cache:
            self._geom_cache[rkey] = torch.full((1, len_q, 1, 2), 0.5, dtype=torch.float32, device=device)
        return self._geom_cache[key] + (self._geom_cache[rkey],)

    def _gated_output(self):
        w, b, g = ps = self.attn.output_proj.weight, self.attn.output_proj.bias, self.gate

        def build():
            t = g.float().tanh()
            return (w.float() * t).to(w.dtype), (b.float() * t).to(b.dtype)
        return self._gated.get(ps, build)

    def project_vision(self, vision_hidden_states):
        return self.attn.project_value(self.norm2(vision_hidden_states))

    def forward(self, hidden_states, vision_hidden_states=None, cross_attention_mask=None, residual=None, inplace=False):
        if records_grad(self, hidden_states, residual, vision_hidden_states if torch.is_tensor(vision_hidden_states) else None):
            return self._forward_training(hidden_states, vision_hidden_states, cross_attention_mask, residual)
        h = self.norm1(hidden_states)
        value = None
        if isinstance(vision_hidden_states, PreparedVision):
            value = vision_hidden_states.values[self.layer_idx]
            _, n_img, hw, _ = vision_hidden_states.raw_shape
            v = None
        else:
            v = self._vision_cache.get_or_build((vision_hidden_states, self.norm2.weight),
                                                lambda: self.norm2(vision_hidden_states), cache=not torch.is_grad_enabled())
            _, n_img, hw, _ = v.shape
        shapes, starts, ref = self._geometry(h.device, n_img, hw, h.shape[1])
        if not torch.is_grad_enabled():
            gw, gb = self._gated_output()
            out = self.attn(query=h, reference_points=ref, input_flatten=v, input_spatial_shapes=shapes,
                            input_level_start_index=starts, input_padding_mask=None, attention_mask=cross_attention_mask,
                            output_weight=gw, output_bias=gb, value=value)
            if residual is None:
                return out
            return residual.add_(out) if inplace else residual + out
        out = self.attn(query=h, reference_points=ref, input_flatten=v, input_spatial_shapes=shapes,
                        input_level_start_index=starts, input_padding_mask=None, attention_mask=cross_attention_mask,
                        value=value)
        gate = self.gate.tanh().to(out.dtype)
        if residual is None:
            return out * gate
        return torch.addcmul(residual, out, gate)

    def _forward_training(self, hidden_states, vision_hidden_states, cross_attention_mask, residual):
        if isinstance(vision_hidden_states, PreparedVision):
            raise RuntimeError("LlamaMMFSAttention under autograd takes the vision feature tensor, not PreparedVision "
                               "(an inference-only cache)")
        h = self.norm1(hidden_states)
        v = self.norm2(vision_hidden_states)
        _, n_img, hw, _ = v.shape
        shapes, starts, ref = self._geometry(h.device, n_img, hw, h.shape[1])
        out = self.attn.forward_differentiable(h, ref, v, shapes, starts, cross_attention_mask)
        out = out * self.gate.tanh().to(out.dtype)
        return out if residual is None else residual + out


class LlamaDecoderLayer(nn.Module):
    def __init__(self, config: LlamaMMFSConfig, use_cross_attn: bool, layer_idx):
        super().__init__()
        self.hidden_size = config.hidden_size
        self.self_attn = LlamaAttention(config=config)
        self.layer_idx = layer_idx
        self.llama_cross_attn = LlamaMMFSAttention(config=config, layer_idx=layer_idx) if use_cross_attn else None
        self.mlp = LlamaMLP(self.hidden_size, config.intermediate_size, config.hidden_act)
        self.input_layernorm = LlamaRMSNorm(config.hidden_size, eps=config.rms_norm_eps)
        self.post_attention_layernorm = LlamaRMSNorm(config.hidden_size, eps=config.rms_norm_eps)

    def forward(self, hidden_states, vision_hidden_states, cross_attention_mask, attention_mask=None,
                position_ids=None, past_key_value=None, output_attentions=False, use_cache=False, inplace=False):
        residual = hidden_states.contiguous()
        inplace = inplace and not torch.is_grad_enabled()
        hidden_states, _, present = self.self_attn(self.input_layernorm(residual), attention_mask=attention_mask,
                                                   position_ids=position_ids, past_key_value=past_key_value,
                                                   use_cache=use_cache, residual=residual, inplace=inplace)
        if self.llama_cross_attn is not None and vision_hidden_states is not None:
            hidden_states = self.llama_cross_attn(hidden_states, vision_hidden_states, cross_attention_mask,
                                                  residual=hidden_states, inplace=inplace)
        hidden_states = self.mlp(self.post_attention_layernorm(hidden_states), residual=hidden_states, inplace=inplace)
        outputs = (hidden_states,)
        if use_cache:
            outputs += (present,)
        return outputs


class LlamaModel(nn.Module):

    def __init__(self, config: LlamaMMFSConfig):
        super().__init__()
        self.config = config
        self.padding_idx = config.pad_token_id
        self.vocab_size = config.vocab_size
        self.cross_attention_frequency = config.cross_attention_frequency
        self.embed_tokens = nn.Embedding(config.vocab_size, config.hidden_size, self.padding_idx)
        use_cross = [i % self.cross_attention_frequency == 0 for i in range(config.num_hidden_layers)]
        self.layers = nn.ModuleList([LlamaDecoderLayer(config, use_cross[i], i) for i in range(config.num_hidden_layers)])
        self.norm = LlamaRMSNorm(config.hidden_size, eps=config.rms_norm_eps)
        self.gradient_checkpointing = False

    def static_cache(self, batch: int, max_len: int, dtype=None, device=None):
        p = self.embed_tokens.weight
        H = self.config.num_attention_heads
        return [StaticKV(batch, max_len, H, self.config.hidden_size // H, dtype or p.dtype, device or p.device)
                for _ in self.layers]

    @torch.no_grad()
    def prepare_vision(self, vision_hidden_states, out: Optional[PreparedVision] = None) -> PreparedVision:
        pv = PreparedVision(vision_hidden_states.shape) if out is None else out
        if tuple(vision_hidden_states.shape) != pv.raw_shape:
            raise RuntimeError(f"prepare_vision: features {tuple(vision_hidden_states.shape)} do not fit {pv.raw_shape}")
        for layer in self.layers:
            if layer.llama_cross_attn is None:
                continue
            val = layer.llama_cross_attn.project_vision(vision_hidden_states)
            if out is None:
                pv.values[layer.layer_idx] = val
            else:
                pv.values[layer.layer_idx].copy_(val)
        return pv

    def get_input_embeddings(self):
        return self.embed_tokens

    def set_input_embeddings(self, value):
        self.embed_tokens = value

    def forward(self, input_ids=None, attention_mask=None, position_ids=None, past_key_values=None,
                inputs_embeds=None, vision_hidden_states=None, cross_attention_mask=None, use_cache=None,
                output_attentions=None, output_hidden_states=None, return_dict=None):
        if use_cache is None:
            grad = records_grad(self, inputs_embeds, vision_hidden_states if torch.is_tensor(vision_hidden_states) else None)
            use_cache = False if grad else self.config.use_cache
        return_dict = True if return_dict is None else return_dict
        if output_attentions:
            raise NotImplementedError("attention probabilities are never materialised")
        if input_ids is not None and inputs_embeds is not None:
            raise ValueError("You cannot specify both decoder_input_ids and decoder_inputs_embeds at the same time")
        if input_ids is None and inputs_embeds is None:
            raise ValueError("You have to specify either decoder_input_ids or decoder_inputs_embeds")
        if inputs_embeds is None:
            inputs_embeds = self.embed_tokens(input_ids)
        B, T, _ = inputs_embeds.shape
        if past_key_values is None:
            past = 0
        else:
            past = past_key_values[0].length if isinstance(past_key_values[0], StaticKV) else past_key_values[0][0].shape[1]
        if position_ids is None:
            position_ids = torch.arange(past, past + T, dtype=torch.long, device=inputs_embeds.device)
        else:
            position_ids = position_ids.view(-1, T).long()
        key_mask = None
        if attention_mask is not None:
            if tuple(attention_mask.shape) != (B, past + T):
                raise ValueError(f"attention_mask should be of size {(B, past + T)}, but is {tuple(attention_mask.shape)}")
            key_mask = attention_mask.to(torch.uint8)

        training = records_grad(self, inputs_embeds, vision_hidden_states if torch.is_tensor(vision_hidden_states) else None)
        if training:
            if use_cache or past_key_values is not None:
                raise RuntimeError("LlamaModel under autograd runs the prefill without a KV cache: pass use_cache=False "
                                   "and no past_key_values, or run under torch.no_grad()")
            check_training_dtype("LlamaModel", inputs_embeds)
        hidden_states = inputs_embeds
        inplace = not torch.is_grad_enabled() and not output_hidden_states
        if inplace:
            hidden_states = hidden_states.clone(memory_format=torch.contiguous_format)
        all_hidden = () if output_hidden_states else None
        next_cache = () if use_cache else None
        for idx, layer in enumerate(self.layers):
            if output_hidden_states:
                all_hidden += (hidden_states,)
            if training and self.gradient_checkpointing:
                outs = torch.utils.checkpoint.checkpoint(layer, hidden_states, vision_hidden_states, cross_attention_mask,
                                                         attention_mask=key_mask, position_ids=position_ids,
                                                         use_reentrant=False)
            else:
                outs = layer(hidden_states, vision_hidden_states, cross_attention_mask, attention_mask=key_mask,
                             position_ids=position_ids,
                             past_key_value=past_key_values[idx] if past_key_values is not None else None,
                             use_cache=use_cache, inplace=inplace)
            hidden_states = outs[0]
            if use_cache:
                next_cache += (outs[1],)
        hidden_states = self.norm(hidden_states)
        if output_hidden_states:
            all_hidden += (hidden_states,)
        if not return_dict:
            return tuple(v for v in [hidden_states, next_cache, all_hidden] if v is not None)
        return SimpleNamespace(last_hidden_state=hidden_states, past_key_values=next_cache, hidden_states=all_hidden,
                               attentions=None)
```

mm-interleaved_b200/ops.py:

```python
from __future__ import annotations

from typing import Optional

import torch

from . import _lib
from .msda import _DTYPE_CODE, _require

launch_counter = [0]


def inference_only(name: str, *tensors) -> None:
    if torch.is_grad_enabled() and any(t is not None and torch.is_tensor(t) and t.requires_grad for t in tensors):
        raise RuntimeError(f"{name}: this kernel is inference-only (no autograd support); call it under torch.no_grad() "
                           "or detach its inputs / freeze its parameters")


def _stream():
    return torch.cuda.current_stream().cuda_stream


def rmsnorm(x: torch.Tensor, weight: torch.Tensor, eps: float) -> torch.Tensor:
    inference_only("rmsnorm", x, weight)
    _require(x.is_cuda and x.is_contiguous() and weight.is_contiguous(), "rmsnorm: contiguous CUDA tensors required")
    _require(weight.dtype == x.dtype and weight.numel() == x.shape[-1], "rmsnorm: weight dtype / size mismatch")
    y = torch.empty_like(x)
    rows = x.numel() // x.shape[-1]
    with torch.cuda.device(x.device):
        rc = _lib.lib().mmfs_rmsnorm(x.data_ptr(), weight.data_ptr(), y.data_ptr(), rows, x.shape[-1], float(eps),
                                     _DTYPE_CODE[x.dtype], _stream())
    _lib.check(rc, "rmsnorm")
    launch_counter[0] += 1
    return y


def layernorm(x: torch.Tensor, weight, bias, eps: float) -> torch.Tensor:
    inference_only("layernorm", x, weight, bias)
    _require(x.is_cuda and x.is_contiguous(), "layernorm: contiguous CUDA tensor required")
    y = torch.empty_like(x)
    rows = x.numel() // x.shape[-1]
    with torch.cuda.device(x.device):
        rc = _lib.lib().mmfs_layernorm(x.data_ptr(), weight.data_ptr() if weight is not None else None,
                                       bias.data_ptr() if bias is not None else None, y.data_ptr(), rows, x.shape[-1],
                                       float(eps), _DTYPE_CODE[x.dtype], _stream())
    _lib.check(rc, "layernorm")
    launch_counter[0] += 1
    return y


def rope_qk_(q: torch.Tensor, k: torch.Tensor, cos: torch.Tensor, sin: torch.Tensor, position_ids: torch.Tensor):
    B, T, H, hd = q.shape
    inference_only("rope_qk_", q, k)
    _require(q.is_cuda and k.shape == q.shape and q.stride(3) == 1 and q.stride(2) == hd and k.stride(3) == 1
             and k.stride(2) == hd and q.stride(0) == T * q.stride(1) and k.stride(0) == T * k.stride(1),
             "rope_qk_: q / k must be (B,T,H,hd) with dense heads and uniform token stride")
    _require(cos.dtype == torch.float32 and sin.dtype == torch.float32 and cos.is_contiguous() and sin.is_contiguous()
             and cos.shape[-1] == hd, "rope_qk_: cos / sin must be contiguous fp32 (max_pos, hd)")
    pos = position_ids.to(torch.int64).contiguous()
    per_batch = 1 if pos.numel() == B * T else 0
    _require(per_batch or pos.numel() == T, "rope_qk_: position_ids must have B*T or T entries")
    with torch.cuda.device(q.device):
        rc = _lib.lib().mmfs_rope_qk(q.data_ptr(), k.data_ptr(), cos.data_ptr(), sin.data_ptr(), pos.data_ptr(),
                                     B * T, T, H, hd, q.stride(1), k.stride(1), per_batch, _DTYPE_CODE[q.dtype], _stream())
    _lib.check(rc, "rope_qk_")
    launch_counter[0] += 1


def rope_qk_append_(q: torch.Tensor, k: torch.Tensor, v: torch.Tensor, cos: torch.Tensor, sin: torch.Tensor,
                    position_ids: torch.Tensor, k_cache: torch.Tensor, v_cache: torch.Tensor, slot) -> None:
    B, T, H, hd = q.shape
    inference_only("rope_qk_append_", q, k, v)
    for t in (q, k, v):
        _require(t.is_cuda and tuple(t.shape) == (B, T, H, hd) and t.stride(3) == 1 and t.stride(2) == hd and
                 t.stride(0) == T * t.stride(1), "rope_qk_append_: q / k / v must be (B,T,H,hd) with dense heads and uniform token stride")
    for c in (k_cache, v_cache):
        _require(c.is_cuda and c.dim() == 4 and c.shape[0] == B and tuple(c.shape[2:]) == (H, hd) and c.stride(3) == 1 and
                 c.stride(2) == hd and c.dtype == q.dtype, "rope_qk_append_: caches must be (B, T_max, H, hd), dense heads")
    _require(k_cache.stride() == v_cache.stride(), "rope_qk_append_: k / v caches must share their strides")
    _require(cos.dtype == torch.float32 and sin.dtype == torch.float32 and cos.is_contiguous() and sin.is_contiguous()
             and cos.shape[-1] == hd, "rope_qk_append_: cos / sin must be contiguous fp32 (max_pos, hd)")
    pos = position_ids.to(torch.int64).contiguous()
    per_batch = 1 if pos.numel() == B * T else 0
    _require(per_batch or pos.numel() == T, "rope_qk_append_: position_ids must have B*T or T entries")
    if isinstance(slot, torch.Tensor):
        _require(slot.is_cuda and slot.dtype == torch.int64 and slot.numel() == 1, "rope_qk_append_: slot tensor must be (1,) int64 on the device")
        slot_dev, slot_host = slot.data_ptr(), 0
    else:
        slot_dev, slot_host = None, int(slot)
        _require(0 <= slot_host and slot_host + T <= k_cache.shape[1], "rope_qk_append_: slot + T exceeds the cache")
    with torch.cuda.device(q.device):
        rc = _lib.lib().mmfs_rope_qk_append(q.data_ptr(), k.data_ptr(), v.data_ptr(), cos.data_ptr(), sin.data_ptr(), pos.data_ptr(),
                                            k_cache.data_ptr(), v_cache.data_ptr(), slot_dev, slot_host, B * T, T, H, hd,
                                            q.stride(1), k.stride(1), v.stride(1), k_cache.stride(0), k_cache.stride(1),
                                            per_batch, _DTYPE_CODE[q.dtype], _stream())
    _lib.check(rc, "rope_qk_append_")
    launch_counter[0] += 1


def decode_select(logits: torch.Tensor, out_ids: torch.Tensor, step: torch.Tensor, finished: torch.Tensor,
                  next_ids: torch.Tensor, params: torch.Tensor, eos: Optional[torch.Tensor] = None, pad_id: int = 0,
                  min_length: int = 0, sample: bool = False, seed: Optional[torch.Tensor] = None,
                  uniforms: Optional[torch.Tensor] = None) -> None:
    inference_only("decode_select", logits)
    _require(logits.is_cuda and logits.dim() == 2 and logits.dtype == torch.float32 and logits.stride(1) == 1,
             "decode_select: logits must be a CUDA fp32 (B, V) tensor with unit column stride")
    B, V = logits.shape
    dev = logits.device
    _require(out_ids.device == dev and out_ids.dtype == torch.int64 and out_ids.dim() == 2 and out_ids.shape[0] == B
             and out_ids.is_contiguous(), "decode_select: out_ids must be contiguous int64 (B, max_new) on the logits' device")
    _require(step.device == dev and step.dtype == torch.int64 and step.numel() == 1, "decode_select: step must be a (1,) int64 device tensor")
    _require(finished.device == dev and finished.dtype in (torch.bool, torch.uint8) and finished.numel() == B
             and finished.is_contiguous(), "decode_select: finished must be contiguous bool / uint8 with B entries")
    _require(next_ids.device == dev and next_ids.dtype == torch.int64 and next_ids.numel() == B and next_ids.is_contiguous(),
             "decode_select: next_ids must be contiguous int64 with B entries")
    _require(params.device == dev and params.dtype == torch.float32 and params.numel() == 3 and params.is_contiguous(),
             "decode_select: params must be a contiguous (3,) fp32 device tensor [repetition_penalty, temperature, top_p]")
    if eos is not None:
        _require(eos.device == dev and eos.dtype == torch.int64 and eos.dim() == 1 and eos.is_contiguous(),
                 "decode_select: eos must be a contiguous 1-D int64 device tensor")
    if seed is not None:
        _require(seed.device == dev and seed.dtype == torch.int64 and seed.numel() == 1, "decode_select: seed must be a (1,) int64 device tensor")
    _require(not sample or seed is not None or uniforms is not None, "decode_select: sampling needs a seed or uniforms")
    if uniforms is not None:
        _require(uniforms.device == dev and uniforms.dtype == torch.float32 and uniforms.numel() == B and uniforms.is_contiguous(),
                 "decode_select: uniforms must be contiguous fp32 with B entries")
    seed_ptr = seed.data_ptr() if seed is not None else None
    with torch.cuda.device(dev):
        rc = _lib.lib().mmfs_decode_select(logits.data_ptr(), logits.stride(0), out_ids.data_ptr(), step.data_ptr(),
                                           finished.data_ptr(), next_ids.data_ptr(), eos.data_ptr() if eos is not None else None,
                                           eos.numel() if eos is not None else 0, int(pad_id), int(min_length),
                                           params.data_ptr(), seed_ptr, uniforms.data_ptr() if uniforms is not None else None,
                                           B, V, out_ids.shape[1], _lib.SELECT_SAMPLE if sample else _lib.SELECT_GREEDY,
                                           _stream())
    _lib.check(rc, "decode_select")
    launch_counter[0] += 1


def beam_candidates(num_beams: int, n_eos: int) -> int:
    return max(2, 1 + n_eos) * num_beams


def beam_select_supported(num_beams: int, n_eos: int, V: int) -> bool:
    return (1 <= num_beams <= _lib.BEAM_MAX_BEAMS and 0 <= n_eos <= _lib.BEAM_MAX_EOS
            and beam_candidates(num_beams, n_eos) <= V <= 1 << 17)


def _check_beam_step(what, logits, step, params, n_params, beam_scores, history, next_ids, parent, done, hyp_scores,
                     hyp_ids, hyp_meta, num_beams, eos):
    inference_only(what, logits)
    _require(logits.is_cuda and logits.dim() == 2 and logits.dtype == torch.float32 and logits.stride(1) == 1,
             f"{what}: logits must be a CUDA fp32 (R, V) tensor with unit column stride")
    R, V = logits.shape
    dev = logits.device
    _require(num_beams > 0 and R % num_beams == 0, f"{what}: the rows must be whole groups of num_beams")
    B = R // num_beams

    def dense(t, name, dtype, shape):
        _require(t.device == dev and t.dtype == dtype and tuple(t.shape) == shape and t.is_contiguous(),
                 f"{what}: {name} must be a contiguous {dtype} {shape} tensor on the logits' device")

    _require(history.dim() == 2, f"{what}: history must be (R, max_new)")
    max_new = history.shape[1]
    dense(step, "step", torch.int64, (1,))
    dense(params, "params", torch.float64, (n_params,))
    dense(beam_scores, "beam_scores", torch.float32, (R,))
    dense(history, "history", torch.int64, (R, max_new))
    dense(next_ids, "next_ids", torch.int64, tuple(next_ids.shape))
    _require(next_ids.numel() == R, f"{what}: next_ids must have R entries")
    dense(parent, "parent", torch.int64, (R,))
    _require(done.device == dev and done.dtype in (torch.bool, torch.uint8) and done.numel() == B and done.is_contiguous(),
             f"{what}: done must be contiguous bool / uint8 with B entries")
    dense(hyp_scores, "hyp_scores", torch.float64, (B, num_beams))
    dense(hyp_ids, "hyp_ids", torch.int64, (B, num_beams, max_new))
    dense(hyp_meta, "hyp_meta", torch.int64, (B, num_beams, 2))
    n_eos = 0
    if eos is not None:
        _require(eos.device == dev and eos.dtype == torch.int64 and eos.dim() == 1 and eos.is_contiguous(),
                 f"{what}: eos must be a contiguous 1-D int64 device tensor")
        n_eos = eos.numel()
    return B, V, max_new, n_eos


def beam_select(logits: torch.Tensor, step: torch.Tensor, params: torch.Tensor, beam_scores: torch.Tensor,
                history: torch.Tensor, next_ids: torch.Tensor, parent: torch.Tensor, done: torch.Tensor,
                hyp_scores: torch.Tensor, hyp_ids: torch.Tensor, hyp_meta: torch.Tensor, scratch: torch.Tensor,
                num_beams: int, eos: Optional[torch.Tensor] = None, pad_id: int = 0, min_length: int = 0) -> None:
    B, V, max_new, n_eos = _check_beam_step("beam_select", logits, step, params, 2, beam_scores, history, next_ids,
                                            parent, done, hyp_scores, hyp_ids, hyp_meta, num_beams, eos)
    R = B * num_beams
    _require(scratch.device == logits.device and scratch.dtype == torch.int64 and scratch.is_contiguous()
             and scratch.numel() >= R * beam_candidates(num_beams, n_eos),
             "beam_select: scratch must be contiguous int64 with R * max(2, 1 + n_eos) * num_beams entries")
    with torch.cuda.device(logits.device):
        rc = _lib.lib().mmfs_beam_select(logits.data_ptr(), logits.stride(0), step.data_ptr(), params.data_ptr(),
                                         beam_scores.data_ptr(), history.data_ptr(), next_ids.data_ptr(), parent.data_ptr(),
                                         done.data_ptr(), hyp_scores.data_ptr(), hyp_ids.data_ptr(), hyp_meta.data_ptr(),
                                         eos.data_ptr() if eos is not None else None, n_eos, int(pad_id), int(min_length),
                                         scratch.data_ptr(), B, num_beams, V, max_new, _stream())
    _lib.check(rc, "beam_select")
    launch_counter[0] += 2


def beam_sample_supported(num_beams: int, n_eos: int, V: int) -> bool:
    return (1 <= num_beams <= _lib.BEAM_MAX_BEAMS and 0 <= n_eos <= _lib.BEAM_MAX_EOS
            and 2 * num_beams <= V <= 1 << 17)


def beam_sample_scratch(num_beams: int, rows: int) -> int:
    return rows * 4 * num_beams


def beam_sample(logits: torch.Tensor, step: torch.Tensor, params: torch.Tensor, beam_scores: torch.Tensor,
                history: torch.Tensor, next_ids: torch.Tensor, parent: torch.Tensor, done: torch.Tensor,
                hyp_scores: torch.Tensor, hyp_ids: torch.Tensor, hyp_meta: torch.Tensor, error: torch.Tensor,
                scratch: torch.Tensor, num_beams: int, eos: Optional[torch.Tensor] = None, pad_id: int = 0,
                min_length: int = 0, top_k: int = 50, seed: Optional[torch.Tensor] = None,
                uniforms: Optional[torch.Tensor] = None) -> None:
    B, V, max_new, n_eos = _check_beam_step("beam_sample", logits, step, params, 4, beam_scores, history, next_ids,
                                            parent, done, hyp_scores, hyp_ids, hyp_meta, num_beams, eos)
    R, dev = B * num_beams, logits.device
    _require(error.device == dev and error.dtype == torch.int32 and error.numel() == 1,
             "beam_sample: error must be a (1,) int32 device tensor")
    _require(scratch.device == dev and scratch.dtype == torch.int64 and scratch.is_contiguous()
             and scratch.numel() >= beam_sample_scratch(num_beams, R),
             "beam_sample: scratch must be contiguous int64 with R * 4 * num_beams entries")
    _require(seed is not None or uniforms is not None, "beam_sample: needs a seed or uniforms")
    if seed is not None:
        _require(seed.device == dev and seed.dtype == torch.int64 and seed.numel() == 1, "beam_sample: seed must be a (1,) int64 device tensor")
    if uniforms is not None:
        _require(uniforms.device == dev and uniforms.dtype == torch.float32 and tuple(uniforms.shape) == (R, V)
                 and uniforms.is_contiguous(), "beam_sample: uniforms must be a contiguous fp32 (R, V) tensor")
    _require(top_k >= 0, "beam_sample: top_k must be >= 0")
    with torch.cuda.device(dev):
        rc = _lib.lib().mmfs_beam_sample(logits.data_ptr(), logits.stride(0), step.data_ptr(), params.data_ptr(),
                                         seed.data_ptr() if seed is not None else None,
                                         uniforms.data_ptr() if uniforms is not None else None, beam_scores.data_ptr(),
                                         history.data_ptr(), next_ids.data_ptr(), parent.data_ptr(), done.data_ptr(),
                                         hyp_scores.data_ptr(), hyp_ids.data_ptr(), hyp_meta.data_ptr(), error.data_ptr(),
                                         eos.data_ptr() if eos is not None else None, n_eos, int(pad_id), int(min_length),
                                         int(top_k), scratch.data_ptr(), B, num_beams, V, max_new, _stream())
    _lib.check(rc, "beam_sample")
    launch_counter[0] += 2


def kv_beam_reorder(kv: torch.Tensor, parent: torch.Tensor, cur: torch.Tensor, step: torch.Tensor, num_beams: int,
                    max_positions: int, done: Optional[torch.Tensor] = None) -> None:
    inference_only("kv_beam_reorder", kv)
    _require(kv.is_cuda and kv.dim() >= 3, "kv_beam_reorder: kv must be a CUDA (n, R, T_max, ...) tensor")
    n, R, T = kv.shape[:3]
    dev = kv.device
    row_bytes = kv[0, 0, 0].numel() * kv.element_size()
    _require(kv[0, 0, 0].is_contiguous() and kv.stride(2) * kv.element_size() >= row_bytes,
             "kv_beam_reorder: each (cache, row, position) entry must be dense")
    _require(num_beams > 0 and R % num_beams == 0, "kv_beam_reorder: the rows must be whole groups of num_beams")
    _require(parent.device == dev and parent.dtype == torch.int64 and parent.numel() == R and parent.is_contiguous(),
             "kv_beam_reorder: parent must be contiguous int64 with R entries")
    for t, name in ((cur, "cur"), (step, "step")):
        _require(t.device == dev and t.dtype == torch.int64 and t.numel() == 1, f"kv_beam_reorder: {name} must be a (1,) int64 device tensor")
    if done is not None:
        _require(done.device == dev and done.dtype in (torch.bool, torch.uint8) and done.numel() == R // num_beams
                 and done.is_contiguous(), "kv_beam_reorder: done must be contiguous bool / uint8 with one entry per group")
    _require(0 < max_positions <= T, "kv_beam_reorder: max_positions must be in [1, T_max]")
    es = kv.element_size()
    with torch.cuda.device(dev):
        rc = _lib.lib().mmfs_kv_beam_reorder(kv.data_ptr(), n, kv.stride(0) * es, R, kv.stride(1) * es, kv.stride(2) * es,
                                             row_bytes, num_beams, parent.data_ptr(), cur.data_ptr(), step.data_ptr(),
                                             done.data_ptr() if done is not None else None, int(max_positions), _stream())
    _lib.check(rc, "kv_beam_reorder")
    launch_counter[0] += 1


def swiglu(gate_up: torch.Tensor) -> torch.Tensor:
    inference_only("swiglu", gate_up)
    _require(gate_up.is_cuda and gate_up.is_contiguous() and gate_up.shape[-1] % 2 == 0, "swiglu: bad input")
    inter = gate_up.shape[-1] // 2
    out = torch.empty(gate_up.shape[:-1] + (inter,), dtype=gate_up.dtype, device=gate_up.device)
    with torch.cuda.device(gate_up.device):
        rc = _lib.lib().mmfs_swiglu(gate_up.data_ptr(), out.data_ptr(), gate_up.numel() // (2 * inter), inter,
                                    _DTYPE_CODE[gate_up.dtype], _stream())
    _lib.check(rc, "swiglu")
    launch_counter[0] += 1
    return out


def geglu(value_gate: torch.Tensor) -> torch.Tensor:
    inference_only("geglu", value_gate)
    _require(value_gate.is_cuda and value_gate.is_contiguous() and value_gate.shape[-1] % 2 == 0, "geglu: bad input")
    inter = value_gate.shape[-1] // 2
    out = torch.empty(value_gate.shape[:-1] + (inter,), dtype=value_gate.dtype, device=value_gate.device)
    with torch.cuda.device(value_gate.device):
        rc = _lib.lib().mmfs_geglu(value_gate.data_ptr(), out.data_ptr(), value_gate.numel() // (2 * inter), inter,
                                   _DTYPE_CODE[value_gate.dtype], _stream())
    _lib.check(rc, "geglu")
    launch_counter[0] += 1
    return out


def attention(q, k, v, key_mask=None, causal=True, past=0, scale=None, force_generic=False) -> torch.Tensor:
    B, Tq, H, hd = q.shape
    Tkv = k.shape[1]
    for t in (q, k, v):
        _require(t.is_cuda and t.stride(3) == 1 and t.stride(2) == hd, "attention: heads must be dense (.., H, hd)")
    inference_only("attention", q, k, v)
    _require(k.shape == v.shape and k.shape[0] == B and k.shape[2] == H and k.shape[3] == hd, "attention: k/v shape mismatch")
    scale = float(scale if scale is not None else hd ** -0.5)
    out = torch.empty((B, Tq, H, hd), dtype=q.dtype, device=q.device)
    km = None
    if key_mask is not None:
        km = key_mask.to(torch.uint8).contiguous()
        _require(tuple(km.shape) == (B, Tkv), "attention: key_mask must be (B, Tkv)")
    from . import attn_tc
    es = q.element_size()
    decode_ok = (Tq == 1 and not force_generic and q.dtype != torch.float64 and hd % 32 == 0 and hd <= 256 and
                 (hd * es) % 16 == 0 and all(t.data_ptr() % 16 == 0 and (t.stride(0) * es) % 16 == 0 and
                                            (t.stride(1) * es) % 16 == 0 for t in (k, v)))
    if not force_generic and attn_tc.supported(q, k, v, Tq, Tkv, hd):
        attn_tc.forward(q, k, v, out, km, causal, past, scale)
    elif decode_ok:
        lib = _lib.lib()
        scratch = torch.empty((lib.mmfs_attn_decode_scratch_floats(B, H, Tkv, hd),), dtype=torch.float32, device=q.device)
        with torch.cuda.device(q.device):
            rc = lib.mmfs_attn_decode(q.data_ptr(), k.data_ptr(), v.data_ptr(), out.data_ptr(),
                                      km.data_ptr() if km is not None else None, scratch.data_ptr(), B, H, Tkv, hd,
                                      q.stride(0), k.stride(0), k.stride(1), v.stride(0), v.stride(1), out.stride(0), scale,
                                      1 if causal else 0, int(past), _DTYPE_CODE[q.dtype], _stream())
        _lib.check(rc, "attention (decode)")
        launch_counter[0] += 1
    else:
        with torch.cuda.device(q.device):
            rc = _lib.lib().mmfs_attn_generic(
                q.data_ptr(), k.data_ptr(), v.data_ptr(), out.data_ptr(), km.data_ptr() if km is not None else None,
                B, H, Tq, Tkv, hd, q.stride(0), q.stride(1), k.stride(0), k.stride(1), v.stride(0), v.stride(1),
                out.stride(0), out.stride(1), scale, 1 if causal else 0, int(past), _DTYPE_CODE[q.dtype], _stream())
        _lib.check(rc, "attention")
    launch_counter[0] += 1
    return out.view(B, Tq, H * hd)



def _check_qkv_view(t, B, T, H, hd, what):
    _require(t.is_cuda and tuple(t.shape) == (B, T, H, hd) and t.stride(3) == 1 and t.stride(2) == hd,
             f"{what}: tensors must be (B, T, H, hd) CUDA views with dense heads")


def attention_forward_lse(q, k, v, key_mask=None, scale=None):
    B, T, H, hd = q.shape
    inference_only("attention_forward_lse", q, k, v)
    for t in (q, k, v):
        _check_qkv_view(t, B, T, H, hd, "attention_forward_lse")
    scale = float(scale if scale is not None else hd ** -0.5)
    out = torch.empty((B, T, H, hd), dtype=q.dtype, device=q.device)
    lse = torch.empty((B, H, T), dtype=torch.float32, device=q.device)
    km = None
    if key_mask is not None:
        km = key_mask.to(torch.uint8).contiguous()
        _require(tuple(km.shape) == (B, T), "attention_forward_lse: key_mask must be (B, T)")
    counter = torch.empty((1,), dtype=torch.int32, device=q.device)
    with torch.cuda.device(q.device):
        rc = _lib.lib().mmfs_attn_forward_lse(
            q.data_ptr(), k.data_ptr(), v.data_ptr(), out.data_ptr(), lse.data_ptr(), km.data_ptr() if km is not None else None,
            B, H, T, T, hd, q.stride(0), q.stride(1), k.stride(0), k.stride(1), v.stride(0), v.stride(1),
            out.stride(0), out.stride(1), scale, 1, 0, _DTYPE_CODE[q.dtype], counter.data_ptr(), _stream())
    _lib.check(rc, "attention_forward_lse")
    launch_counter[0] += 1
    return out, lse


def attention_backward(q, k, v, out, d_out, lse, dq, dk, dv, key_mask=None, scale=None) -> None:
    B, T, H, hd = q.shape
    inference_only("attention_backward", q, k, v, out, d_out)
    for t in (q, k, v, out, d_out, dq, dk, dv):
        _check_qkv_view(t, B, T, H, hd, "attention_backward")
    _require(all(t.dtype == q.dtype for t in (k, v, out, d_out, dq, dk, dv)), "attention_backward: dtype mismatch")
    _require(lse.dtype == torch.float32 and tuple(lse.shape) == (B, H, T) and lse.is_contiguous(),
             "attention_backward: lse must be contiguous fp32 (B, H, T)")
    scale = float(scale if scale is not None else hd ** -0.5)
    km = None
    if key_mask is not None:
        km = key_mask.to(torch.uint8).contiguous()
        _require(tuple(km.shape) == (B, T), "attention_backward: key_mask must be (B, T)")
    delta = torch.empty((B, H, T), dtype=torch.float32, device=q.device)
    with torch.cuda.device(q.device):
        rc = _lib.lib().mmfs_attn_backward(
            q.data_ptr(), k.data_ptr(), v.data_ptr(), out.data_ptr(), d_out.data_ptr(), lse.data_ptr(), dq.data_ptr(),
            dk.data_ptr(), dv.data_ptr(), delta.data_ptr(), km.data_ptr() if km is not None else None, B, H, T, hd,
            q.stride(0), q.stride(1), k.stride(0), k.stride(1), v.stride(0), v.stride(1), out.stride(0), out.stride(1),
            d_out.stride(0), d_out.stride(1), dq.stride(0), dq.stride(1), dk.stride(0), dk.stride(1), dv.stride(0),
            dv.stride(1), scale, _DTYPE_CODE[q.dtype], _stream())
    _lib.check(rc, "attention_backward")
    launch_counter[0] += 3


def rmsnorm_backward(x: torch.Tensor, weight: torch.Tensor, dy: torch.Tensor, eps: float, weight_grad: bool = True):
    inference_only("rmsnorm_backward", x, weight, dy)
    _require(x.is_cuda and x.is_contiguous() and dy.is_contiguous() and weight.is_contiguous() and dy.shape == x.shape,
             "rmsnorm_backward: contiguous CUDA tensors of one shape required")
    _require(weight.dtype == x.dtype == dy.dtype and weight.numel() == x.shape[-1], "rmsnorm_backward: weight dtype / size mismatch")
    cols = x.shape[-1]
    rows = x.numel() // cols
    dx = torch.empty_like(x)
    dw = torch.empty_like(weight) if weight_grad else None
    partials = (torch.empty((min(rows, _lib.RMSNORM_BWD_PARTS), cols), dtype=torch.float32, device=x.device)
                if weight_grad else None)
    with torch.cuda.device(x.device):
        rc = _lib.lib().mmfs_rmsnorm_backward(x.data_ptr(), weight.data_ptr(), dy.data_ptr(), dx.data_ptr(),
                                              dw.data_ptr() if dw is not None else None,
                                              partials.data_ptr() if partials is not None else None, rows, cols, float(eps),
                                              _DTYPE_CODE[x.dtype], _stream())
    _lib.check(rc, "rmsnorm_backward")
    launch_counter[0] += 2 if weight_grad else 1
    return dx, dw


def swiglu_backward(gate_up: torch.Tensor, d_out: torch.Tensor) -> torch.Tensor:
    inference_only("swiglu_backward", gate_up, d_out)
    _require(gate_up.is_cuda and gate_up.is_contiguous() and d_out.is_contiguous() and gate_up.shape[-1] % 2 == 0
             and d_out.shape == gate_up.shape[:-1] + (gate_up.shape[-1] // 2,) and d_out.dtype == gate_up.dtype,
             "swiglu_backward: bad input")
    inter = gate_up.shape[-1] // 2
    d_gu = torch.empty_like(gate_up)
    with torch.cuda.device(gate_up.device):
        rc = _lib.lib().mmfs_swiglu_backward(gate_up.data_ptr(), d_out.data_ptr(), d_gu.data_ptr(),
                                             gate_up.numel() // (2 * inter), inter, _DTYPE_CODE[gate_up.dtype], _stream())
    _lib.check(rc, "swiglu_backward")
    launch_counter[0] += 1
    return d_gu


def conv2d_supported(x: torch.Tensor, weight: torch.Tensor, stride: int, padding: int) -> bool:
    if x.dtype not in (torch.bfloat16, torch.float16) or not x.is_cuda or x.dim() != 4:
        return False
    B, Cin, H, W = x.shape
    Cout, _, KH, KW = weight.shape
    Ho, Wo = (H + 2 * padding - KH) // stride + 1, (W + 2 * padding - KW) // stride + 1
    tile = (Wo % 16 == 0 and Ho % 8 == 0) or (Wo == 8 and Ho == 8 and B % 2 == 0)
    return Cin % 64 == 0 and (Cout % 160 == 0 or Cout % 128 == 0) and stride in (1, 2) and tile


def conv2d(x: torch.Tensor, weight_khwc: torch.Tensor, bias=None, stride: int = 1, padding: int = 0, add_bc=None,
           residual=None) -> torch.Tensor:
    B, Cin, H, W = x.shape
    Cout, KH, KW, _ = weight_khwc.shape
    inference_only("conv2d", x, weight_khwc, bias, add_bc, residual)
    _require(x.is_contiguous(memory_format=torch.channels_last) and weight_khwc.is_contiguous(), "conv2d: x must be channels_last")
    Ho, Wo = (H + 2 * padding - KH) // stride + 1, (W + 2 * padding - KW) // stride + 1
    out = torch.empty((B, Cout, Ho, Wo), dtype=x.dtype, device=x.device, memory_format=torch.channels_last)
    if residual is not None:
        _require(residual.shape == out.shape and residual.is_contiguous(memory_format=torch.channels_last), "conv2d: residual layout")
    if add_bc is not None:
        add_bc = add_bc.contiguous()
    with torch.cuda.device(x.device):
        rc = _lib.lib().mmfs_conv2d_nhwc(
            x.data_ptr(), weight_khwc.data_ptr(), bias.data_ptr() if bias is not None else None,
            add_bc.data_ptr() if add_bc is not None else None, residual.data_ptr() if residual is not None else None,
            out.data_ptr(), B, H, W, Cin, Cout, KH, KW, stride, padding, _DTYPE_CODE[x.dtype], _stream())
    _lib.check(rc, "conv2d")
    launch_counter[0] += 1
    return out


def fold_up2x_weights(weight: torch.Tensor) -> torch.Tensor:
    acc = torch.float64 if weight.dtype == torch.float64 else torch.float32
    fold = torch.tensor([[[1, 0, 0], [0, 1, 1]], [[1, 1, 0], [0, 0, 1]]], dtype=acc, device=weight.device)
    w = torch.einsum("pak,ockl,qbl->pqoabc", fold, weight.to(acc), fold)
    return w.reshape(4, *w.shape[2:]).to(weight.dtype).contiguous()


def conv2d_up2x_supported(x: torch.Tensor, weight: torch.Tensor) -> bool:
    if x.dtype not in (torch.bfloat16, torch.float16) or not x.is_cuda or x.dim() != 4 or tuple(weight.shape[2:]) != (3, 3):
        return False
    B, Cin, H, W = x.shape
    Cout = weight.shape[0]
    tile = (W % 16 == 0 and H % 8 == 0) or (W == 8 and H == 8 and B % 2 == 0)
    return Cin % 64 == 0 and (Cout % 160 == 0 or Cout % 128 == 0) and tile


def conv2d_up2x(x: torch.Tensor, weight_phases: torch.Tensor, bias=None) -> torch.Tensor:
    B, Cin, H, W = x.shape
    Cout = weight_phases.shape[1]
    inference_only("conv2d_up2x", x, weight_phases, bias)
    _require(x.is_contiguous(memory_format=torch.channels_last) and weight_phases.is_contiguous(), "conv2d_up2x: x must be channels_last")
    _require(tuple(weight_phases.shape) == (4, Cout, 2, 2, Cin), "conv2d_up2x: weights must be (4, Cout, 2, 2, Cin)")
    out = torch.empty((B, Cout, 2 * H, 2 * W), dtype=x.dtype, device=x.device, memory_format=torch.channels_last)
    with torch.cuda.device(x.device):
        rc = _lib.lib().mmfs_conv2d_up2x_nhwc(x.data_ptr(), weight_phases.data_ptr(), bias.data_ptr() if bias is not None else None,
                                              out.data_ptr(), B, H, W, Cin, Cout, _DTYPE_CODE[x.dtype], _stream())
    _lib.check(rc, "conv2d_up2x")
    launch_counter[0] += 1
    return out


def conv2d_down2x_supported(x: torch.Tensor, weight: torch.Tensor) -> bool:
    if x.dtype not in (torch.bfloat16, torch.float16) or not x.is_cuda or x.dim() != 4 or tuple(weight.shape[2:]) != (3, 3):
        return False
    B, Cin, H, W = x.shape
    Cout = weight.shape[0]
    if H % 2 or W % 2:
        return False
    Ho, Wo = H // 2, W // 2
    tile = (Wo % 16 == 0 and Ho % 8 == 0) or (Wo == 8 and Ho == 8 and B % 2 == 0)
    return Cin % 64 == 0 and (Cout % 160 == 0 or Cout % 128 == 0) and tile


def conv2d_down2x(x: torch.Tensor, weight_khwc: torch.Tensor, bias=None) -> torch.Tensor:
    B, Cin, H, W = x.shape
    Cout = weight_khwc.shape[0]
    inference_only("conv2d_down2x", x, weight_khwc, bias)
    _require(x.is_contiguous(memory_format=torch.channels_last) and weight_khwc.is_contiguous(), "conv2d_down2x: x must be channels_last")
    _require(tuple(weight_khwc.shape) == (Cout, 3, 3, Cin), "conv2d_down2x: weights must be (Cout, 3, 3, Cin)")
    out = torch.empty((B, Cout, H // 2, W // 2), dtype=x.dtype, device=x.device, memory_format=torch.channels_last)
    with torch.cuda.device(x.device):
        rc = _lib.lib().mmfs_conv2d_down2x_nhwc(x.data_ptr(), weight_khwc.data_ptr(), bias.data_ptr() if bias is not None else None,
                                                out.data_ptr(), B, H, W, Cin, Cout, _DTYPE_CODE[x.dtype], _stream())
    _lib.check(rc, "conv2d_down2x")
    launch_counter[0] += 1
    return out


def group_norm_supported(x: torch.Tensor) -> bool:
    if not x.is_cuda or x.dim() != 4 or x.dtype not in _DTYPE_CODE or x.dtype == torch.float64:
        return False
    vec = 16 // x.element_size()
    return x.shape[1] % vec == 0 and x.shape[1] // vec <= 1024 and x.is_contiguous(memory_format=torch.channels_last)


def group_norm_nhwc(x: torch.Tensor, groups: int, weight=None, bias=None, eps: float = 1e-5, silu: bool = False) -> torch.Tensor:
    inference_only("group_norm_nhwc", x, weight, bias)
    _require(group_norm_supported(x), "group_norm_nhwc: need a CUDA channels_last f32/f16/bf16 tensor with C % (16/size) == 0")
    B, C, H, W = x.shape
    y = torch.empty_like(x, memory_format=torch.channels_last)
    stats = torch.empty((B, 64, groups, 2), dtype=torch.float32, device=x.device)
    with torch.cuda.device(x.device):
        rc = _lib.lib().mmfs_groupnorm_nhwc(x.data_ptr(), weight.data_ptr() if weight is not None else None,
                                            bias.data_ptr() if bias is not None else None, y.data_ptr(), stats.data_ptr(),
                                            B, H * W, C, groups, float(eps), int(silu), _DTYPE_CODE[x.dtype], _stream())
    _lib.check(rc, "group_norm_nhwc")
    launch_counter[0] += 2
    return y
```

Baseline: 2.668.

## Fuse gate/up projection GEMM with SwiGLU epilogue in warp-specialized TMA kernel

After: 2.683, median of 6. Within noise of the previous version (+0.6%).

```diff
diff --git a/include/mmfs_b200.h b/include/mmfs_b200.h
--- a/include/mmfs_b200.h
+++ b/include/mmfs_b200.h
@@ -113,6 +113,15 @@
 int mmfs_conv2d_nhwc(const void *x, const void *w, const void *bias, const void *add_bc, const void *residual, void *out,
                      int B, int H, int W, int Cin, int Cout, int KH, int KW, int stride, int pad, int dtype, void *stream);
 
+int mmfs_linear_supported(long M, int N, int K, int dtype);
+int mmfs_linear_swiglu_supported(long M, int inter, int K, int dtype);
+int mmfs_linear_rope_qkv_supported(long M, int H, int hd, int K, int dtype);
+int mmfs_linear(const void *x, const void *w, void *out, long M, int N, int K, int dtype, void *stream);
+int mmfs_linear_swiglu(const void *x, const void *w_gate_up, void *act, long M, int inter, int K, int dtype, void *stream);
+int mmfs_linear_rope_qkv(const void *x, const void *w_qkv, void *qkv, const float *cos_table, const float *sin_table,
+                         const int64_t *position_ids, long M, int T_len, int H, int hd, int K, int pos_per_batch,
+                         int dtype, void *stream);
+
 int mmfs_conv2d_up2x_nhwc(const void *x, const void *w_phases, const void *bias, void *out, int B, int H, int W, int Cin,
                           int Cout, int dtype, void *stream);
 
diff --git a/mm-interleaved_b200/_lib.py b/mm-interleaved_b200/_lib.py
--- a/mm-interleaved_b200/_lib.py
+++ b/mm-interleaved_b200/_lib.py
@@ -39,6 +39,12 @@
     "mmfs_groupnorm_nhwc": (_I, [_P] * 5 + [_I] * 4 + [_F, _I, _I, _P]),
     "mmfs_conv2d_nhwc": (_I, [_P] * 6 + [_I] * 10 + [_P]),
     "mmfs_conv2d_up2x_nhwc": (_I, [_P] * 4 + [_I] * 6 + [_P]),
+    "mmfs_linear_supported": (_I, [_L, _I, _I, _I]),
+    "mmfs_linear_swiglu_supported": (_I, [_L, _I, _I, _I]),
+    "mmfs_linear_rope_qkv_supported": (_I, [_L, _I, _I, _I, _I]),
+    "mmfs_linear": (_I, [_P, _P, _P, _L, _I, _I, _I, _P]),
+    "mmfs_linear_swiglu": (_I, [_P, _P, _P, _L, _I, _I, _I, _P]),
+    "mmfs_linear_rope_qkv": (_I, [_P] * 6 + [_L] + [_I] * 6 + [_P]),
     "mmfs_conv2d_down2x_nhwc": (_I, [_P] * 4 + [_I] * 6 + [_P]),
     "mmfs_attn_decode_scratch_floats": (_L, [_I] * 4),
     "mmfs_attn_decode": (_I, [_P] * 6 + [_I] * 4 + [_L] * 6 + [_F, _I, _I, _I, _P]),
diff --git a/mm-interleaved_b200/csrc/conv_igemm_sm100.cu b/mm-interleaved_b200/csrc/conv_igemm_sm100.cu
--- a/mm-interleaved_b200/csrc/conv_igemm_sm100.cu
+++ b/mm-interleaved_b200/csrc/conv_igemm_sm100.cu
@@ -14,15 +14,6 @@
     int tiles_w, tiles_h;
 };
 
-template <typename T> __device__ __forceinline__ uint32_t cpack2(float a, float b);
-template <> __device__ __forceinline__ uint32_t cpack2<__nv_bfloat16>(float a, float b) {
-    __nv_bfloat162 t = __floats2bfloat162_rn(a, b);
-    return *reinterpret_cast<uint32_t *>(&t);
-}
-template <> __device__ __forceinline__ uint32_t cpack2<__half>(float a, float b) {
-    __half2 t = __floats2half2_rn(a, b);
-    return *reinterpret_cast<uint32_t *>(&t);
-}
 template <typename T> __device__ __forceinline__ float2 cunpack2(const T *p);
 template <> __device__ __forceinline__ float2 cunpack2<__nv_bfloat16>(const __nv_bfloat16 *p) {
     return __bfloat1622float2(*reinterpret_cast<const __nv_bfloat162 *>(p));
diff --git a/mm-interleaved_b200/csrc/linear_fused_sm100.cu b/mm-interleaved_b200/csrc/linear_fused_sm100.cu
--- /dev/null
+++ b/mm-interleaved_b200/csrc/linear_fused_sm100.cu
@@ -0,0 +1,254 @@
+#include "llama_epi.cuh"
+#include "tc_common.cuh"
+
+namespace mmfs {
+
+constexpr int kLinBM = 128, kLinBN = 256, kLinBK = 64, kLinStages = 4;
+constexpr int kLinThreads = 384;
+constexpr int kLinGroupM = 16;
+constexpr int kLinStageBytes = (kLinBM + kLinBN) * kLinBK * 2;
+constexpr size_t kLinSmem = (size_t)kLinStages * kLinStageBytes + 2 * kLinStages * 8;
+enum { kEpiPlain = 0, kEpiSwiglu = 1, kEpiRope = 2 };
+
+struct LinParams {
+    void *out;
+    int M, N, K;
+    const float *cos_t, *sin_t;
+    const int64_t *pos;
+    int T_len, pos_per_batch, rot_cols;
+};
+
+template <int R> __device__ __forceinline__ void reg_alloc() { asm volatile("setmaxnreg.inc.sync.aligned.u32 %0;" ::"n"(R)); }
+template <int R> __device__ __forceinline__ void reg_release() { asm volatile("setmaxnreg.dec.sync.aligned.u32 %0;" ::"n"(R)); }
+
+__device__ __forceinline__ void lin_tile(int t, int tiles_m, int tiles_n, int &tm, int &tn) {
+    const int group = kLinGroupM * tiles_n;
+    const int g = t / group, first = g * kLinGroupM;
+    const int gm = min(tiles_m - first, kLinGroupM);
+    const int r = t - g * group;
+    tm = first + r % gm;
+    tn = r / gm;
+}
+
+template <typename T, int EPI>
+__device__ __forceinline__ void lin_epilogue(const float (&acc)[128], const LinParams &p, int row0, int n0, int tq) {
+#pragma unroll
+    for (int i = 0; i < 2; ++i) {
+        const int row = row0 + 8 * i;
+        if (row >= p.M) continue;
+        if constexpr (EPI == kEpiSwiglu) {
+            T *op = static_cast<T *>(p.out) + (size_t)row * (p.N / 2) + n0 / 2 + 2 * tq;
+#pragma unroll
+            for (int j = 0; j < 16; ++j) {
+                const int g = 4 * j + 2 * i, u = 4 * (j + 16) + 2 * i;
+                const float o0 = glu_out<T, 0>(rnd<T>(acc[g]), rnd<T>(acc[u]));
+                const float o1 = glu_out<T, 0>(rnd<T>(acc[g + 1]), rnd<T>(acc[u + 1]));
+                *reinterpret_cast<uint32_t *>(op + 8 * j) = cpack2<T>(o0, o1);
+            }
+        } else {
+            T *op = static_cast<T *>(p.out) + (size_t)row * p.N + n0 + 2 * tq;
+            if (EPI == kEpiRope && n0 < p.rot_cols) {
+                const long ps = p.pos[p.pos_per_batch ? row : row % p.T_len];
+                const float *cp = p.cos_t + ps * 128 + 2 * tq, *sp = p.sin_t + ps * 128 + 2 * tq;
+#pragma unroll
+                for (int j = 0; j < 8; ++j) {
+                    const float2 c = *reinterpret_cast<const float2 *>(cp + 8 * j);
+                    const float2 s = *reinterpret_cast<const float2 *>(sp + 8 * j);
+                    const float cs[2] = {rnd<T>(c.x), rnd<T>(c.y)}, sn[2] = {rnd<T>(s.x), rnd<T>(s.y)};
+#pragma unroll
+                    for (int h = 0; h < 2; ++h) {
+                        const int a = 16 * h + j, b = a + 8;
+                        float o1[2], o2[2];
+#pragma unroll
+                        for (int c2 = 0; c2 < 2; ++c2)
+                            rope_pair<T>(rnd<T>(acc[4 * a + 2 * i + c2]), rnd<T>(acc[4 * b + 2 * i + c2]), cs[c2], sn[c2], o1[c2], o2[c2]);
+                        *reinterpret_cast<uint32_t *>(op + 8 * a) = cpack2<T>(o1[0], o1[1]);
+                        *reinterpret_cast<uint32_t *>(op + 8 * b) = cpack2<T>(o2[0], o2[1]);
+                    }
+                }
+            } else {
+#pragma unroll
+                for (int j = 0; j < 32; ++j)
+                    *reinterpret_cast<uint32_t *>(op + 8 * j) = cpack2<T>(acc[4 * j + 2 * i], acc[4 * j + 2 * i + 1]);
+            }
+        }
+    }
+}
+
+template <typename T, int EPI>
+__global__ void __launch_bounds__(kLinThreads, 1)
+linear_kernel(const __grid_constant__ CUtensorMap map_x, const __grid_constant__ CUtensorMap map_w, const LinParams p) {
+    constexpr uint32_t A_BYTES = kLinBM * 128;
+    extern __shared__ __align__(1024) uint8_t smem_raw[];
+    if ((s_addr(smem_raw) & 1023u) != 0u) { asm volatile("trap;"); }
+    uint64_t *full = reinterpret_cast<uint64_t *>(smem_raw + kLinStages * kLinStageBytes), *empty = full + kLinStages;
+
+    const int warp = threadIdx.x >> 5, lane = threadIdx.x & 31;
+    const int tiles_m = (p.M + kLinBM - 1) / kLinBM, tiles_n = p.N / kLinBN, n_tiles = tiles_m * tiles_n;
+    const int n_k = p.K / kLinBK;
+
+    if (threadIdx.x == 0) {
+        for (int i = 0; i < kLinStages; ++i) { bar_init(full + i, 1); bar_init(empty + i, 8); }
+        asm volatile("fence.mbarrier_init.release.cluster;" ::: "memory");
+    }
+    __syncthreads();
+
+    if (warp < 4) {
+        reg_release<40>();
+        if (threadIdx.x == 0) {
+            int it = 0;
+            for (int t = blockIdx.x; t < n_tiles; t += gridDim.x) {
+                int tm, tn;
+                lin_tile(t, tiles_m, tiles_n, tm, tn);
+                for (int kt = 0; kt < n_k; ++kt, ++it) {
+                    const int s = it % kLinStages;
+                    bar_wait(empty + s, ((it / kLinStages) & 1) ^ 1);
+                    uint8_t *sa = smem_raw + s * kLinStageBytes;
+                    bar_expect_tx(full + s, kLinStageBytes);
+                    tma_load_2d(sa, &map_x, full + s, kt * kLinBK, tm * kLinBM);
+                    tma_load_2d(sa + A_BYTES, &map_w, full + s, kt * kLinBK, tn * kLinBN);
+                }
+            }
+        }
+        return;
+    }
+
+    reg_alloc<232>();
+    const int wg = (warp >> 2) - 1;
+    float acc[128];
+    int it = 0;
+    for (int t = blockIdx.x; t < n_tiles; t += gridDim.x) {
+        int tm, tn;
+        lin_tile(t, tiles_m, tiles_n, tm, tn);
+        for (int kt = 0; kt < n_k; ++kt, ++it) {
+            const int s = it % kLinStages;
+            bar_wait(full + s, (it / kLinStages) & 1);
+            const uint32_t sa = s_addr(smem_raw) + s * kLinStageBytes;
+            reg_fence(acc);
+            wgmma_fence();
+#pragma unroll
+            for (int kk = 0; kk < 4; ++kk) {
+                const uint64_t da = smem_desc(sa + wg * 64 * 128 + kk * 32, 16, 1024), db = smem_desc(sa + A_BYTES + kk * 32, 16, 1024);
+                Wgmma<T>::ss_n256(acc, da, db, (kt | kk) != 0);
+            }
+            wgmma_commit();
+            wgmma_wait<1>();
+            reg_fence(acc);
+            if (kt > 0 && lane == 0) bar_arrive(empty + (it - 1) % kLinStages);
+        }
+        wgmma_wait<0>();
+        reg_fence(acc);
+        if (lane == 0) bar_arrive(empty + (it - 1) % kLinStages);
+        lin_epilogue<T, EPI>(acc, p, tm * kLinBM + wg * 64 + (warp & 3) * 16 + (lane >> 2), tn * kLinBN, lane & 3);
+    }
+}
+
+}
+
+using namespace mmfs;
+
+namespace {
+
+bool lin_shape_ok(long M, int N, int K, int dtype) {
+    return (dtype == MMFS_BF16 || dtype == MMFS_F16) && M > 0 && M <= 0x7fffffffL - kLinBM && N > 0 && K > 0 &&
+           N % kLinBN == 0 && K % kLinBK == 0 && (M + kLinBM - 1) / kLinBM * (long)(N / kLinBN) <= 0x7fffffffL;
+}
+
+bool rope_shape_ok(int H, int hd, int K, int dtype) {
+    return hd == 128 && H > 0 && H % 2 == 0 && lin_shape_ok(1, 3 * H * hd, K, dtype);
+}
+
+template <auto kern>
+int launch(int grid, cudaStream_t st, const CUtensorMap &mx, const CUtensorMap &mw, const LinParams &p) {
+    const int rc = ensure_dynamic_smem<kern>(kLinSmem);
+    if (rc != MMFS_OK) return rc;
+    kern<<<grid, kLinThreads, kLinSmem, st>>>(mx, mw, p);
+    MMFS_CUDA(cudaGetLastError());
+    return MMFS_OK;
+}
+
+template <int EPI>
+int launch_linear(const char *what, const void *x, const void *w, LinParams p, int dtype, void *stream) {
+    if (!lin_shape_ok(p.M, p.N, p.K, dtype) || ((uintptr_t)x | (uintptr_t)w | (uintptr_t)p.out) % 16 != 0) {
+        set_error("%s: needs bf16/f16, N %% 256 == 0, K %% 64 == 0, 16-byte aligned pointers (M=%d N=%d K=%d)", what, p.M, p.N,
+                  p.K);
+        return MMFS_EUNSUPPORTED;
+    }
+    EncodeTiledFn enc = tensor_map_encoder();
+    if (!enc) { set_error("%s: cuTensorMapEncodeTiled unavailable", what); return MMFS_ECUDA; }
+    const CUtensorMapDataType dt = dtype == MMFS_BF16 ? CU_TENSOR_MAP_DATA_TYPE_BFLOAT16 : CU_TENSOR_MAP_DATA_TYPE_FLOAT16;
+    CUtensorMap mx, mw;
+    const cuuint64_t strides[1] = {(cuuint64_t)p.K * 2};
+    const cuuint32_t estr[2] = {1, 1};
+    {
+        const cuuint64_t dims[2] = {(cuuint64_t)p.K, (cuuint64_t)p.M};
+        const cuuint32_t box[2] = {kLinBK, kLinBM};
+        CUresult r = enc(&mx, dt, 2, const_cast<void *>(x), dims, strides, box, estr, CU_TENSOR_MAP_INTERLEAVE_NONE,
+                         CU_TENSOR_MAP_SWIZZLE_128B, CU_TENSOR_MAP_L2_PROMOTION_L2_256B, CU_TENSOR_MAP_FLOAT_OOB_FILL_NONE);
+        if (r != CUDA_SUCCESS) { set_error("%s: tensor map (x) failed (%d)", what, (int)r); return MMFS_ECUDA; }
+    }
+    {
+        const cuuint64_t dims[2] = {(cuuint64_t)p.K, (cuuint64_t)p.N};
+        const cuuint32_t box[2] = {kLinBK, kLinBN};
+        CUresult r = enc(&mw, dt, 2, const_cast<void *>(w), dims, strides, box, estr, CU_TENSOR_MAP_INTERLEAVE_NONE,
+                         CU_TENSOR_MAP_SWIZZLE_128B, CU_TENSOR_MAP_L2_PROMOTION_L2_256B, CU_TENSOR_MAP_FLOAT_OOB_FILL_NONE);
+        if (r != CUDA_SUCCESS) { set_error("%s: tensor map (w) failed (%d)", what, (int)r); return MMFS_ECUDA; }
+    }
+    const long tiles = (p.M + kLinBM - 1) / kLinBM * (long)(p.N / kLinBN);
+    const int grid = (int)(tiles < num_sms() ? tiles : num_sms());
+    cudaStream_t st = (cudaStream_t)stream;
+    return dispatch_dtype<kF16Types>(dtype, what, [&](auto tag) {
+        using T = typename decltype(tag)::type;
+        return launch<linear_kernel<T, EPI>>(grid, st, mx, mw, p);
+    });
+}
+
+LinParams lin_params(void *out, long M, int N, int K) {
+    LinParams p = {};
+    p.out = out; p.M = (int)M; p.N = N; p.K = K;
+    return p;
+}
+
+}
+
+extern "C" int mmfs_linear_supported(long M, int N, int K, int dtype) { return lin_shape_ok(M, N, K, dtype) ? 1 : 0; }
+
+extern "C" int mmfs_linear_swiglu_supported(long M, int inter, int K, int dtype) {
+    return inter > 0 && inter % 128 == 0 && lin_shape_ok(M, 2 * inter, K, dtype) ? 1 : 0;
+}
+
+extern "C" int mmfs_linear_rope_qkv_supported(long M, int H, int hd, int K, int dtype) {
+    return M > 0 && rope_shape_ok(H, hd, K, dtype) && lin_shape_ok(M, 3 * H * hd, K, dtype) ? 1 : 0;
+}
+
+extern "C" int mmfs_linear(const void *x, const void *w, void *out, long M, int N, int K, int dtype, void *stream) {
+    MMFS_CHECK_ARG(M > 0 && N > 0 && K > 0, "linear: bad dimension");
+    MMFS_CHECK_ARG(x && w && out, "linear: null pointer argument");
+    return launch_linear<kEpiPlain>("linear", x, w, lin_params(out, M, N, K), dtype, stream);
+}
+
+extern "C" int mmfs_linear_swiglu(const void *x, const void *w_gate_up, void *act, long M, int inter, int K, int dtype,
+                                  void *stream) {
+    MMFS_CHECK_ARG(M > 0 && inter > 0 && K > 0, "linear_swiglu: bad dimension");
+    MMFS_CHECK_ARG(x && w_gate_up && act, "linear_swiglu: null pointer argument");
+    if (inter % 128 != 0) {
+        set_error("linear_swiglu: inter %% 128 != 0 (inter=%d)", inter);
+        return MMFS_EUNSUPPORTED;
+    }
+    return launch_linear<kEpiSwiglu>("linear_swiglu", x, w_gate_up, lin_params(act, M, 2 * inter, K), dtype, stream);
+}
+
+extern "C" int mmfs_linear_rope_qkv(const void *x, const void *w_qkv, void *qkv, const float *cos_table, const float *sin_table,
+                                    const int64_t *position_ids, long M, int T_len, int H, int hd, int K, int pos_per_batch,
+                                    int dtype, void *stream) {
+    MMFS_CHECK_ARG(M > 0 && T_len > 0 && H > 0 && hd > 0 && K > 0, "linear_rope_qkv: bad dimension");
+    MMFS_CHECK_ARG(x && w_qkv && qkv && cos_table && sin_table && position_ids, "linear_rope_qkv: null pointer argument");
+    if (!rope_shape_ok(H, hd, K, dtype)) {
+        set_error("linear_rope_qkv: needs hd = 128, even H, K %% 64 == 0, bf16/f16 (H=%d hd=%d K=%d)", H, hd, K);
+        return MMFS_EUNSUPPORTED;
+    }
+    LinParams p = lin_params(qkv, M, 3 * H * hd, K);
+    p.cos_t = cos_table; p.sin_t = sin_table; p.pos = position_ids;
+    p.T_len = T_len; p.pos_per_batch = pos_per_batch; p.rot_cols = 2 * H * hd;
+    return launch_linear<kEpiRope>("linear_rope_qkv", x, w_qkv, p, dtype, stream);
+}
diff --git a/mm-interleaved_b200/csrc/llama_epi.cuh b/mm-interleaved_b200/csrc/llama_epi.cuh
--- /dev/null
+++ b/mm-interleaved_b200/csrc/llama_epi.cuh
@@ -0,0 +1,25 @@
+#pragma once
+#include "common.cuh"
+
+namespace mmfs {
+
+template <typename T> __device__ __forceinline__ float rnd(float x) { return to_op(from_op<T>(x)); }
+template <> __device__ __forceinline__ float rnd<float>(float x) { return x; }
+
+template <typename T> __device__ __forceinline__ float silu_op(float g) { return __fdividef(g, 1.f + __expf(-g)); }
+template <> __device__ __forceinline__ float silu_op<float>(float g) { return g / (1.f + expf(-g)); }
+
+template <typename T, int ACT> __device__ __forceinline__ float glu_act(float g) {
+    if (ACT == 0) return silu_op<T>(g);
+    return 0.5f * g * (1.f + erff(g * 0.70710678118654752f));
+}
+
+template <typename T, int ACT> __device__ __forceinline__ float glu_out(float g, float u) { return rnd<T>(glu_act<T, ACT>(g)) * u; }
+
+template <typename T>
+__device__ __forceinline__ void rope_pair(float x1, float x2, float cs, float sn, float &o1, float &o2) {
+    o1 = rnd<T>(x1 * cs) + rnd<T>(-x2 * sn);
+    o2 = rnd<T>(x2 * cs) + rnd<T>(x1 * sn);
+}
+
+}
diff --git a/mm-interleaved_b200/csrc/llama_ops_sm100.cu b/mm-interleaved_b200/csrc/llama_ops_sm100.cu
--- a/mm-interleaved_b200/csrc/llama_ops_sm100.cu
+++ b/mm-interleaved_b200/csrc/llama_ops_sm100.cu
@@ -1,9 +1,7 @@
 #include "common.cuh"
+#include "llama_epi.cuh"
 
 namespace mmfs {
-
-template <typename T> __device__ __forceinline__ float rnd(float x) { return to_op(from_op<T>(x)); }
-template <> __device__ __forceinline__ float rnd<float>(float x) { return x; }
 
 __device__ __forceinline__ float block_sum(float v, float *s_red) {
 #pragma unroll
@@ -211,10 +209,7 @@
             Vec16<T>::unpack(v1, x1);
             Vec16<T>::unpack(v2, x2);
 #pragma unroll
-            for (int i = 0; i < VEC; ++i) {
-                o1[i] = rnd<T>(x1[i] * cs[i]) + rnd<T>(-x2[i] * sn[i]);
-                o2[i] = rnd<T>(x2[i] * cs[i]) + rnd<T>(x1[i] * sn[i]);
-            }
+            for (int i = 0; i < VEC; ++i) rope_pair<T>(x1[i], x2[i], cs[i], sn[i], o1[i], o2[i]);
             *reinterpret_cast<uint4 *>(x) = Vec16<T>::pack(o1);
             *reinterpret_cast<uint4 *>(x + half) = Vec16<T>::pack(o2);
         }
@@ -262,22 +257,11 @@
             Vec16<T>::unpack(*reinterpret_cast<const uint4 *>(src), x1);
             Vec16<T>::unpack(*reinterpret_cast<const uint4 *>(src + half), x2);
 #pragma unroll
-            for (int i = 0; i < VEC; ++i) {
-                o1[i] = rnd<T>(x1[i] * cs[i]) + rnd<T>(-x2[i] * sn[i]);
-                o2[i] = rnd<T>(x2[i] * cs[i]) + rnd<T>(x1[i] * sn[i]);
-            }
+            for (int i = 0; i < VEC; ++i) rope_pair<T>(x1[i], x2[i], cs[i], sn[i], o1[i], o2[i]);
             *reinterpret_cast<uint4 *>(dst) = Vec16<T>::pack(o1);
             *reinterpret_cast<uint4 *>(dst + half) = Vec16<T>::pack(o2);
         }
     }
-}
-
-template <typename T> __device__ __forceinline__ float silu_op(float g) { return __fdividef(g, 1.f + __expf(-g)); }
-template <> __device__ __forceinline__ float silu_op<float>(float g) { return g / (1.f + expf(-g)); }
-
-template <typename T, int ACT> __device__ __forceinline__ float glu_act(float g) {
-    if (ACT == 0) return silu_op<T>(g);
-    return 0.5f * g * (1.f + erff(g * 0.70710678118654752f));
 }
 
 template <typename T, int ACT = 0, bool GATE_SECOND = false>
@@ -296,18 +280,18 @@
             float g[VEC], u[VEC], o[VEC];
             Vec16<T>::unpack(g0, g); Vec16<T>::unpack(u0, u);
 #pragma unroll
-            for (int k = 0; k < VEC; ++k) o[k] = rnd<T>(glu_act<T, ACT>(g[k])) * u[k];
+            for (int k = 0; k < VEC; ++k) o[k] = glu_out<T, ACT>(g[k], u[k]);
             stg_v4(o_row + i * VEC, Vec16<T>::pack(o));
             Vec16<T>::unpack(g1, g); Vec16<T>::unpack(u1, u);
 #pragma unroll
-            for (int k = 0; k < VEC; ++k) o[k] = rnd<T>(glu_act<T, ACT>(g[k])) * u[k];
+            for (int k = 0; k < VEC; ++k) o[k] = glu_out<T, ACT>(g[k], u[k]);
             stg_v4(o_row + j * VEC, Vec16<T>::pack(o));
         }
         if (i < nvec) {
             float g[VEC], u[VEC], o[VEC];
             Vec16<T>::unpack(ldg_nc_v4(g_row + i * VEC), g); Vec16<T>::unpack(ldg_nc_v4(u_row + i * VEC), u);
 #pragma unroll
-            for (int k = 0; k < VEC; ++k) o[k] = rnd<T>(glu_act<T, ACT>(g[k])) * u[k];
+            for (int k = 0; k < VEC; ++k) o[k] = glu_out<T, ACT>(g[k], u[k]);
             stg_v4(o_row + i * VEC, Vec16<T>::pack(o));
         }
     }
diff --git a/mm-interleaved_b200/csrc/tc_common.cuh b/mm-interleaved_b200/csrc/tc_common.cuh
--- a/mm-interleaved_b200/csrc/tc_common.cuh
+++ b/mm-interleaved_b200/csrc/tc_common.cuh
@@ -52,6 +52,14 @@
             : "l"(da), "l"(db), "r"(acc)); \
     } \
      \
+    __device__ __forceinline__ static void ss_n256(float (&d)[128], uint64_t da, uint64_t db, int acc) { \
+        asm volatile( \
+            "{\n\t.reg .pred p;\n\tsetp.ne.b32 p, %130, 0;\n\t" \
+            "wgmma.mma_async.sync.aligned.m64n256k16.f32." TY "." TY " {%0,%1,%2,%3,%4,%5,%6,%7,%8,%9,%10,%11,%12,%13,%14,%15,%16,%17,%18,%19,%20,%21,%22,%23,%24,%25,%26,%27,%28,%29,%30,%31,%32,%33,%34,%35,%36,%37,%38,%39,%40,%41,%42,%43,%44,%45,%46,%47,%48,%49,%50,%51,%52,%53,%54,%55,%56,%57,%58,%59,%60,%61,%62,%63,%64,%65,%66,%67,%68,%69,%70,%71,%72,%73,%74,%75,%76,%77,%78,%79,%80,%81,%82,%83,%84,%85,%86,%87,%88,%89,%90,%91,%92,%93,%94,%95,%96,%97,%98,%99,%100,%101,%102,%103,%104,%105,%106,%107,%108,%109,%110,%111,%112,%113,%114,%115,%116,%117,%118,%119,%120,%121,%122,%123,%124,%125,%126,%127}, %128, %129, p, 1, 1, 0, 0;\n\t}" \
+            : "+f"(d[0]), "+f"(d[1]), "+f"(d[2]), "+f"(d[3]), "+f"(d[4]), "+f"(d[5]), "+f"(d[6]), "+f"(d[7]), "+f"(d[8]), "+f"(d[9]), "+f"(d[10]), "+f"(d[11]), "+f"(d[12]), "+f"(d[13]), "+f"(d[14]), "+f"(d[15]), "+f"(d[16]), "+f"(d[17]), "+f"(d[18]), "+f"(d[19]), "+f"(d[20]), "+f"(d[21]), "+f"(d[22]), "+f"(d[23]), "+f"(d[24]), "+f"(d[25]), "+f"(d[26]), "+f"(d[27]), "+f"(d[28]), "+f"(d[29]), "+f"(d[30]), "+f"(d[31]), "+f"(d[32]), "+f"(d[33]), "+f"(d[34]), "+f"(d[35]), "+f"(d[36]), "+f"(d[37]), "+f"(d[38]), "+f"(d[39]), "+f"(d[40]), "+f"(d[41]), "+f"(d[42]), "+f"(d[43]), "+f"(d[44]), "+f"(d[45]), "+f"(d[46]), "+f"(d[47]), "+f"(d[48]), "+f"(d[49]), "+f"(d[50]), "+f"(d[51]), "+f"(d[52]), "+f"(d[53]), "+f"(d[54]), "+f"(d[55]), "+f"(d[56]), "+f"(d[57]), "+f"(d[58]), "+f"(d[59]), "+f"(d[60]), "+f"(d[61]), "+f"(d[62]), "+f"(d[63]), "+f"(d[64]), "+f"(d[65]), "+f"(d[66]), "+f"(d[67]), "+f"(d[68]), "+f"(d[69]), "+f"(d[70]), "+f"(d[71]), "+f"(d[72]), "+f"(d[73]), "+f"(d[74]), "+f"(d[75]), "+f"(d[76]), "+f"(d[77]), "+f"(d[78]), "+f"(d[79]), "+f"(d[80]), "+f"(d[81]), "+f"(d[82]), "+f"(d[83]), "+f"(d[84]), "+f"(d[85]), "+f"(d[86]), "+f"(d[87]), "+f"(d[88]), "+f"(d[89]), "+f"(d[90]), "+f"(d[91]), "+f"(d[92]), "+f"(d[93]), "+f"(d[94]), "+f"(d[95]), "+f"(d[96]), "+f"(d[97]), "+f"(d[98]), "+f"(d[99]), "+f"(d[100]), "+f"(d[101]), "+f"(d[102]), "+f"(d[103]), "+f"(d[104]), "+f"(d[105]), "+f"(d[106]), "+f"(d[107]), "+f"(d[108]), "+f"(d[109]), "+f"(d[110]), "+f"(d[111]), "+f"(d[112]), "+f"(d[113]), "+f"(d[114]), "+f"(d[115]), "+f"(d[116]), "+f"(d[117]), "+f"(d[118]), "+f"(d[119]), "+f"(d[120]), "+f"(d[121]), "+f"(d[122]), "+f"(d[123]), "+f"(d[124]), "+f"(d[125]), "+f"(d[126]), "+f"(d[127]) \
+            : "l"(da), "l"(db), "r"(acc)); \
+    } \
+     \
     __device__ __forceinline__ static void rs_n64(float (&d)[32], const uint32_t (&a)[4], uint64_t db, int acc) { \
         asm volatile( \
             "{\n\t.reg .pred p;\n\tsetp.ne.b32 p, %37, 0;\n\t" \
@@ -71,6 +79,16 @@
 template <> struct Wgmma<__half> { MMFS_WGMMA_OPS("f16") };
 #undef MMFS_WGMMA_OPS
 
+
+template <typename T> __device__ __forceinline__ uint32_t cpack2(float a, float b);
+template <> __device__ __forceinline__ uint32_t cpack2<__nv_bfloat16>(float a, float b) {
+    __nv_bfloat162 t = __floats2bfloat162_rn(a, b);
+    return *reinterpret_cast<uint32_t *>(&t);
+}
+template <> __device__ __forceinline__ uint32_t cpack2<__half>(float a, float b) {
+    __half2 t = __floats2half2_rn(a, b);
+    return *reinterpret_cast<uint32_t *>(&t);
+}
 
 __device__ __forceinline__ void tma_load_2d(void *dst, const CUtensorMap *map, uint64_t *bar, int c0, int c1) {
     asm volatile(
diff --git a/mm-interleaved_b200/llama_mmfs.py b/mm-interleaved_b200/llama_mmfs.py
--- a/mm-interleaved_b200/llama_mmfs.py
+++ b/mm-interleaved_b200/llama_mmfs.py
@@ -97,6 +97,26 @@
         return self._cache.get(ws, lambda: torch.cat(ws, 0).contiguous())
 
 
+USE_FUSED_LINEARS = True
+FUSED_MIN_ROWS = 1024
+
+
+def _fused_rows(x) -> bool:
+    return (USE_FUSED_LINEARS and x.is_cuda and x.dtype in (torch.bfloat16, torch.float16)
+            and x.numel() // x.shape[-1] >= FUSED_MIN_ROWS)
+
+
+class _InterleavedGateUp:
+
+    def __init__(self, gate, up):
+        self.linears = (gate, up)
+        self._cache = WeightCache()
+
+    def get(self):
+        ws = [l.weight for l in self.linears]
+        return self._cache.get(ws, lambda: ops.interleave_gate_up(torch.cat(ws, 0)))
+
+
 def _addmm_residual(residual, x, weight, inplace):
     r2 = residual.view(-1, residual.shape[-1])
     x2 = x.reshape(-1, x.shape[-1])
@@ -115,6 +135,7 @@
         self.down_proj = nn.Linear(intermediate_size, hidden_size, bias=False)
         self.up_proj = nn.Linear(hidden_size, intermediate_size, bias=False)
         self._gate_up = _CatWeight(self.gate_proj, self.up_proj)
+        self._gate_up_il = _InterleavedGateUp(self.gate_proj, self.up_proj)
 
     def forward(self, x, residual=None, inplace=False):
         if records_grad(self, x, residual):
@@ -123,8 +144,10 @@
             if residual is None:
                 return self.down_proj(act)
             return _addmm_residual(residual, act, self.down_proj.weight, False)
-        gu = F.linear(x, self._gate_up.get())
-        act = ops.swiglu(gu)
+        if _fused_rows(x) and x.is_contiguous() and ops.linear_swiglu_supported(x, self.gate_proj.out_features):
+            act = ops.linear_swiglu(x, self._gate_up_il.get())
+        else:
+            act = ops.swiglu(F.linear(x, self._gate_up.get()))
         if residual is None:
             return self.down_proj(act)
         return _addmm_residual(residual, act, self.down_proj.weight, inplace)
diff --git a/mm-interleaved_b200/ops.py b/mm-interleaved_b200/ops.py
--- a/mm-interleaved_b200/ops.py
+++ b/mm-interleaved_b200/ops.py
@@ -427,6 +427,92 @@
     return d_gu
 
 
+GATE_UP_BLOCK = 128
+
+
+def interleave_gate_up(gate_up: torch.Tensor) -> torch.Tensor:
+    n2, K = gate_up.shape
+    _require(n2 % (2 * GATE_UP_BLOCK) == 0, "interleave_gate_up: intermediate size must be a multiple of 128")
+    nb = n2 // (2 * GATE_UP_BLOCK)
+    return gate_up.view(2, nb, GATE_UP_BLOCK, K).transpose(0, 1).reshape(n2, K).contiguous()
+
+
+def deinterleave_gate_up(w: torch.Tensor) -> torch.Tensor:
+    n2, K = w.shape
+    _require(n2 % (2 * GATE_UP_BLOCK) == 0, "deinterleave_gate_up: intermediate size must be a multiple of 128")
+    nb = n2 // (2 * GATE_UP_BLOCK)
+    return w.view(nb, 2, GATE_UP_BLOCK, K).transpose(0, 1).reshape(n2, K).contiguous()
+
+
+def _rows(x: torch.Tensor) -> int:
+    return x.numel() // x.shape[-1]
+
+
+def linear_supported(x: torch.Tensor, n: int) -> bool:
+    return x.dtype in _DTYPE_CODE and bool(_lib.lib().mmfs_linear_supported(_rows(x), n, x.shape[-1], _DTYPE_CODE[x.dtype]))
+
+
+def linear_swiglu_supported(x: torch.Tensor, inter: int) -> bool:
+    return x.dtype in _DTYPE_CODE and bool(
+        _lib.lib().mmfs_linear_swiglu_supported(_rows(x), inter, x.shape[-1], _DTYPE_CODE[x.dtype]))
+
+
+def linear_rope_qkv_supported(x: torch.Tensor, heads: int, head_dim: int) -> bool:
+    return x.dtype in _DTYPE_CODE and bool(
+        _lib.lib().mmfs_linear_rope_qkv_supported(_rows(x), heads, head_dim, x.shape[-1], _DTYPE_CODE[x.dtype]))
+
+
+def _check_linear(what, x, w):
+    _require(x.is_cuda and x.is_contiguous() and w.is_contiguous() and w.dim() == 2 and w.shape[1] == x.shape[-1]
+             and w.dtype == x.dtype, f"{what}: x (..., K) and weight (N, K) must be contiguous CUDA tensors of one dtype")
+
+
+def linear(x: torch.Tensor, weight: torch.Tensor) -> torch.Tensor:
+    inference_only("linear", x, weight)
+    _check_linear("linear", x, weight)
+    out = torch.empty(x.shape[:-1] + (weight.shape[0],), dtype=x.dtype, device=x.device)
+    with torch.cuda.device(x.device):
+        rc = _lib.lib().mmfs_linear(x.data_ptr(), weight.data_ptr(), out.data_ptr(), _rows(x), weight.shape[0], x.shape[-1],
+                                    _DTYPE_CODE[x.dtype], _stream())
+    _lib.check(rc, "linear")
+    launch_counter[0] += 1
+    return out
+
+
+def linear_swiglu(x: torch.Tensor, w_gate_up_interleaved: torch.Tensor) -> torch.Tensor:
+    inference_only("linear_swiglu", x, w_gate_up_interleaved)
+    _check_linear("linear_swiglu", x, w_gate_up_interleaved)
+    inter = w_gate_up_interleaved.shape[0] // 2
+    out = torch.empty(x.shape[:-1] + (inter,), dtype=x.dtype, device=x.device)
+    with torch.cuda.device(x.device):
+        rc = _lib.lib().mmfs_linear_swiglu(x.data_ptr(), w_gate_up_interleaved.data_ptr(), out.data_ptr(), _rows(x), inter,
+                                           x.shape[-1], _DTYPE_CODE[x.dtype], _stream())
+    _lib.check(rc, "linear_swiglu")
+    launch_counter[0] += 1
+    return out
+
+
+def linear_rope_qkv(x: torch.Tensor, w_qkv: torch.Tensor, cos: torch.Tensor, sin: torch.Tensor, position_ids: torch.Tensor,
+                    heads: int, head_dim: int) -> torch.Tensor:
+    B, T, _ = x.shape
+    inference_only("linear_rope_qkv", x, w_qkv)
+    _check_linear("linear_rope_qkv", x, w_qkv)
+    _require(w_qkv.shape[0] == 3 * heads * head_dim, "linear_rope_qkv: weight must be (3*H*hd, K)")
+    _require(cos.dtype == torch.float32 and sin.dtype == torch.float32 and cos.is_contiguous() and sin.is_contiguous()
+             and cos.shape[-1] == head_dim, "linear_rope_qkv: cos / sin must be contiguous fp32 (max_pos, hd)")
+    pos = position_ids.to(torch.int64).contiguous()
+    per_batch = 1 if pos.numel() == B * T else 0
+    _require(per_batch or pos.numel() == T, "linear_rope_qkv: position_ids must have B*T or T entries")
+    out = torch.empty((B, T, 3, heads, head_dim), dtype=x.dtype, device=x.device)
+    with torch.cuda.device(x.device):
+        rc = _lib.lib().mmfs_linear_rope_qkv(x.data_ptr(), w_qkv.data_ptr(), out.data_ptr(), cos.data_ptr(), sin.data_ptr(),
+                                             pos.data_ptr(), B * T, T, heads, head_dim, x.shape[-1], per_batch,
+                                             _DTYPE_CODE[x.dtype], _stream())
+    _lib.check(rc, "linear_rope_qkv")
+    launch_counter[0] += 1
+    return out
+
+
 def conv2d_supported(x: torch.Tensor, weight: torch.Tensor, stride: int, padding: int) -> bool:
     if x.dtype not in (torch.bfloat16, torch.float16) or not x.is_cuda or x.dim() != 4:
         return False
```
